# polli-labs/linnaeus

Hardware: AMD Instinct MI355X
Metric: images/sec (train fwd+bwd) mFormerV1_sm 3x224x224 (higher is better)
Workload: dtype bf16; 1 GPU; mFormerV1_sm train step (forward + 4-task CE loss + backward + AdamW (one HIP launch)), bf16 operands / fp32 accumulate+residual, batch 256/GPU, 3x224x224 synthetic, DropPath 0.2, gradient checkpointing off; per_gpu_batch=256, global_batch=256, parallelism=dp1, grad_mode=direct

## Files before the change

include/lnx.h:

```cpp
#ifndef LNX_H
#define LNX_H
#include <stdint.h>

#ifdef __cplusplus
extern "C" {
#endif

#define LNX_F32 0
#define LNX_BF16 1

const char* lnx_last_error(void);
int lnx_version(void);
int lnx_device_cus(void);
int lnx_set_cu_margin(int cus);

typedef struct lnx_rowmap {
    int group, pad, off;
} lnx_rowmap;

enum { LNX_ACT_NONE = 0, LNX_ACT_GELU = 1, LNX_ACT_RELU = 2, LNX_ACT_GELU_BWD = 3, LNX_ACT_RELU_BWD = 4,
       LNX_ACT_GELU_D = 5, LNX_ACT_MUL_AUX = 6 };
enum { LNX_ADDR_PLAIN = 0, LNX_ADDR_PATCH2 = 1 };

typedef struct lnx_gemm_args {
// ... 9 lines not shown
    int a_mode, Hin, Win, Cin;
    int c_mode;
    lnx_rowmap c_map;
    const float* bias;
    void* c2;
    int64_t ldc2;
    int act;
    const void* aux;
    int64_t ldaux;
    const float* gamma;
    const float* rowscale;
    int rows_per_sample;
    const float* res;
    int64_t ldres;
    void* c8;
    int64_t ldc8;
    void* c8_scales;
} lnx_gemm_args;

int lnx_gemm_nt(const lnx_gemm_args* args, void* stream);

#define LNX_GEMM_GROUP_MAX 8
int lnx_gemm_nt_group_ok(const lnx_gemm_args* problems, int n, int accumulate);
int lnx_gemm_nt_group(const lnx_gemm_args* problems, int n, int accumulate, void* stream);

enum { LNX_NT_KERNEL_NONE = 0, LNX_NT_KERNEL_V1 = 1 , LNX_NT_KERNEL_V2 = 2 ,
       LNX_NT_KERNEL_SKINNY = 3 , LNX_NT_KERNEL_V4 = 4 ,
       LNX_NT_KERNEL_FP8 = 6 , LNX_NT_KERNEL_V7 = 7 ,
       LNX_NT_KERNEL_MX8 = 8 , LNX_NT_KERNEL_V9 = 9 ,
       LNX_NT_KERNEL_EXPERIMENT = 15 , LNX_NT_KERNEL_KINDS = 16 };
int lnx_last_nt_kernel(void);
int64_t lnx_nt_kernel_launches(int kind);
int lnx_nt_dispatch(const lnx_gemm_args* args);

int lnx_amax(const void* x, int x_dtype, int64_t ldx, int rows, int cols, float* amax, void* stream);
int lnx_quantize_fp8(const void* x, int x_dtype, int64_t ldx, int rows, int cols, const float* amax, void* y, int64_t ldy, float* scale_out, void* stream);
int lnx_gemm_nt_fp8(const lnx_gemm_args* args, const float* a_scale, const float* w_scale, void* stream);

int lnx_quantize_mxfp8(const void* x, int x_dtype, int64_t ldx, int rows, int cols, void* y, int64_t ldy, void* scales, void* stream);
int lnx_gemm_nt_mxfp8(const lnx_gemm_args* args, const void* a_scales, const void* w_scales, void* stream);

typedef struct lnx_wgrad_args {
    int dtype;
    int M, N, K;
    const void* dY;
    int64_t lddy;
    const void* A;
    int64_t lda;
    int a_mode, Hin, Win, Cin;
    float* dW;
    int64_t lddw;
    int k_perm_c;
    float* db;
    int splits;
    int k_store;
    float* ws;
    int64_t ws_floats;
    int defer;
} lnx_wgrad_args;
#define LNX_TN_WS_FLOATS (256 * (256 * 128 + 256))

int lnx_gemm_tn(const lnx_wgrad_args* args, void* stream);
int lnx_gemm_tn_flush(void* stream);
int lnx_gemm_tn_discard(void);


// ... 52 lines not shown
    void* dx2_8_scales;
    int64_t lddx2_8;
    int defer;
} lnx_ln_bwd_args;
int lnx_layernorm_bwd(const lnx_ln_bwd_args* args, void* stream);
int lnx_layernorm_bwd_flush(void* stream);
int lnx_layernorm_bwd_discard(void);

enum { LNX_LN_COLS_NONE = 0 , LNX_LN_COLS_ATOMICS = 1 ,
       LNX_LN_COLS_WORKSPACE = 2  };
typedef struct lnx_ln_launch {
    int G;
    int V;
    int pair;
    int full;
    int mx;
    int grid;
    int cols;
    int slices;
} lnx_ln_launch;
int lnx_layernorm_fwd_query(const lnx_ln_args* args, lnx_ln_launch* out);
int lnx_layernorm_bwd_query(const lnx_ln_bwd_args* args, lnx_ln_launch* out);

typedef struct lnx_dwconv_args {
    int B, H, W, C;
    const void* x;
    int x_dtype;
    const float* w49;
    const float* bias;
    int flip;
    const float* res;
    void* y;
    int y_dtype;
} lnx_dwconv_args;
int lnx_dwconv7_fwd(const lnx_dwconv_args* args, void* stream);

typedef struct lnx_dwconv_wgrad_args {
    int B, H, W, C;
    const void* x;
    int x_dtype;
    const void* dy;
    int dy_dtype;
    float* dw;
    float* db;
} lnx_dwconv_wgrad_args;
int lnx_dwconv7_wgrad(const lnx_dwconv_wgrad_args* args, void* stream);

enum { LNX_ROPE_COS = 0, LNX_ROPE_ROTATE = 1 };
int lnx_rope_cos_table(const float* freqs , int heads, int H, int W, float* cos_out ,
                       float* dsin_out ,
                       void* stream);
int lnx_rope_cos_table_hd(const float* freqs, int heads, int head_dim, int H, int W, float* cos_out, float* dsin_out, void* stream);
int lnx_rope_cossin_table_hd(const float* freqs, int heads, int head_dim, int H, int W, float* cos_out, float* sin_out, float* dsin_out, void* stream);
#define LNX_ROPE_TABLES_MAX 24
typedef struct {
    const float* freqs;
    float* cos_out;
    float* dsin_out;
    int heads, H, W;
    int head_dim;
    int rope_mode;
    float* sin_out;
} lnx_rope_table;
int lnx_rope_cos_tables(const lnx_rope_table* tables, int n, void* stream);
int64_t lnx_attn_bwd_ws_floats(int B, int N, int heads);
int64_t lnx_attn_bwd_ws_floats_hd(int B, int N, int heads, int head_dim);
// ... 448 lines not shown
    void* ln_out;
    float* mean;
    float* rstd;
} lnx_convmlp_args;
int lnx_convmlp_fwd(const lnx_convmlp_args* args, void* stream);

typedef struct lnx_convmlp_bwd_args {
    int dtype, M, C;
    const float* g;
    const void* ln;
    const void* z;
    const void* w1;
    const float* b1;
    const void* w2t;
    const void* w1t;
    const float* gamma;
    const float* rowscale;
    int rows_per_sample;
    void* act;
    void* dh;
    void* dz;
    void* dln;
    float* dgamma;
    const void* y;
    const float* ln_w;
    const float* mean;
    const float* rstd;
    float* d_ln_w;
    float* d_ln_b;
    float* ws;
    int64_t ws_floats;
    int dz_plain;
    int ln_defer;
} lnx_convmlp_bwd_args;
int lnx_convmlp_bwd(const lnx_convmlp_bwd_args* args, void* stream);
int64_t lnx_convmlp_bwd_ws_floats(int C, int M);


#define LNX_MAX_META 8
#define LNX_MAX_TASKS 16
typedef struct lnx_mformer_cfg {
    int dtype;
    int batch, img_h, img_w, in_chans;
    int dims[4];
    int conv_depths[2];
    int rope_depths[2];
    int rope_heads[2];
    int mlp_hidden[2];
    int n_meta;
    int meta_dims[LNX_MAX_META];
    int only_last_cls;
    int n_tasks;
    int task_classes[LNX_MAX_TASKS];
    int inference;
    int recompute;
    int fp8;
    int rope_mode;
} lnx_mformer_cfg;

typedef struct lnx_plan lnx_plan;
int lnx_plan_create(const lnx_mformer_cfg* cfg, lnx_plan** out);
void lnx_plan_destroy(lnx_plan* p);
int64_t lnx_plan_workspace_bytes(const lnx_plan* p);
int lnx_plan_num_params(const lnx_plan* p);
const char* lnx_plan_param_name(const lnx_plan* p, int i);
int64_t lnx_plan_param_numel(const lnx_plan* p, int i);
// ... 28 lines not shown
```

linnaeus_amd/_lib.py:

```python
from __future__ import annotations

import ctypes as C
import os

_HERE = os.path.dirname(os.path.abspath(__file__))
LIB_PATH = os.environ.get("LNX_LIB_PATH") or os.path.join(_HERE, "liblnx_hip.so")

F32, BF16 = 0, 1
ACT_NONE, ACT_GELU, ACT_RELU, ACT_GELU_BWD, ACT_RELU_BWD, ACT_GELU_D, ACT_MUL_AUX = 0, 1, 2, 3, 4, 5, 6
TN_WS_FLOATS = 256 * (256 * 128 + 256)
ADDR_PLAIN, ADDR_PATCH2 = 0, 1


class LnxError(RuntimeError):
    pass


class RowMap(C.Structure):
    _fields_ = [("group", C.c_int), ("pad", C.c_int), ("off", C.c_int)]


class GemmArgs(C.Structure):
    _fields_ = [
        ("dtype", C.c_int), ("M", C.c_int), ("N", C.c_int), ("K", C.c_int),
# ... 199 lines not shown
            _lib.lnx_resize_coeffs.argtypes = [C.c_int, C.c_int, C.c_int, C.c_void_p, C.c_void_p]
            _lib.lnx_preprocess_scratch_bytes.argtypes = [C.POINTER(PreprocessImage), C.c_int, C.c_int, C.c_int, C.c_int]
            _lib.lnx_preprocess_scratch_bytes.restype = C.c_int64
            _lib.lnx_preprocess.argtypes = [C.POINTER(PreprocessArgs), C.c_void_p]
            _lib.lnx_preprocess.restype = C.c_int
        if hasattr(_lib, "lnx_meta_mask"):
            _lib.lnx_meta_mask.argtypes = [C.POINTER(MetaMaskArgs), C.c_void_p]
            _lib.lnx_meta_mask.restype = C.c_int
        if hasattr(_lib, "lnx_layernorm_fwd_query"):
            _lib.lnx_layernorm_fwd_query.argtypes = [C.POINTER(LnArgs), C.POINTER(LnLaunch)]
            _lib.lnx_layernorm_bwd_query.argtypes = [C.POINTER(LnBwdArgs), C.POINTER(LnLaunch)]
        older = bool(os.environ.get("LNX_LIB_PATH")) and os.environ.get("LNX_LIB_OLDER") == "1"
        for name in EXPORTS:
            if not hasattr(_lib, name) and not older:
                raise LnxError(f"{LIB_PATH} does not export {name}; rebuild it")
    return _lib


def check(rc: int, what: str) -> None:
    if rc != 0:
        raise LnxError(f"{what} failed (rc={rc}): {lib().lnx_last_error().decode()}")


AUG_CLAMP, AUG_POSTERIZE, AUG_SOLARIZE, AUG_SOLARIZE_ADD, AUG_INVERT, AUG_BRIGHTNESS, AUG_CONTRAST = range(7)

NT_KERNEL_NONE, NT_KERNEL_V1, NT_KERNEL_V2, NT_KERNEL_SKINNY, NT_KERNEL_V4, NT_KERNEL_FP8, NT_KERNEL_V7, NT_KERNEL_MX8, NT_KERNEL_V9, NT_KERNEL_EXPERIMENT = 0, 1, 2, 3, 4, 6, 7, 8, 9, 15

ROPE_COS, ROPE_ROTATE = 0, 1

ATTN_KERNEL_NONE, ATTN_KERNEL_RES4, ATTN_KERNEL_RES8, ATTN_KERNEL_TILED4, ATTN_KERNEL_TILED8 = range(5)

EXPORTS = [
    "lnx_last_error", "lnx_version", "lnx_device_cus", "lnx_set_cu_margin",
    "lnx_gemm_nt", "lnx_last_nt_kernel", "lnx_nt_kernel_launches", "lnx_nt_dispatch", "lnx_gemm_tn", "lnx_gemm_tn_flush", "lnx_gemm_tn_discard", "lnx_amax", "lnx_quantize_fp8", "lnx_gemm_nt_fp8", "lnx_quantize_mxfp8", "lnx_gemm_nt_mxfp8", "lnx_dropout_mul", "lnx_dropout_residual", "lnx_plan_dropout_bytes", "lnx_plan_set_dropout", "lnx_plan_attn_dropout_bytes", "lnx_plan_set_attn_dropout",
    "lnx_layernorm_fwd", "lnx_layernorm_bwd", "lnx_layernorm_bwd_flush", "lnx_layernorm_bwd_discard", "lnx_layernorm_fwd_query", "lnx_layernorm_bwd_query",
    "lnx_dwconv7_fwd", "lnx_dwconv7_wgrad",
    "lnx_gemm_nt_group_ok", "lnx_gemm_nt_group", "lnx_rope_cos_table", "lnx_rope_cos_table_hd", "lnx_rope_cossin_table_hd", "lnx_rope_cos_tables", "lnx_attn_bwd_ws_floats", "lnx_attn_bwd_ws_floats_hd", "lnx_attn_fwd", "lnx_attn_bwd", "lnx_attn_bwd_flush", "lnx_attn_bwd_discard", "lnx_attn_dispatch", "lnx_last_attn_kernel", "lnx_last_attn_bwd_launches",
    "lnx_im2col_stem", "lnx_scale_cast", "lnx_layerscale_bwd", "lnx_layerscale_apply_wgrad", "lnx_fill_rows", "lnx_colsum_rows",
    "lnx_agg2_fwd", "lnx_agg2_bwd", "lnx_pack_meta", "lnx_meta_heads_supported", "lnx_meta_heads_fwd", "lnx_meta_heads_bwd", "lnx_meta_heads_bwd_part_floats", "lnx_prep_weights", "lnx_prep_blocks", "lnx_softce", "lnx_softce_multi", "lnx_stem_fwd", "lnx_stem_fwd_ok", "lnx_adamw_blocks", "lnx_grad_sumsq", "lnx_adamw_step", "lnx_ademamix_step", "lnx_muon_layout", "lnx_muon_step", "lnx_muon_launches", "lnx_gradnorm_sumsq", "lnx_gradnorm_update",
    "lnx_metrics_table_sizes", "lnx_metrics_update", "lnx_predict", "lnx_resize_taps", "lnx_resize_coeffs", "lnx_preprocess_scratch_bytes", "lnx_preprocess", "lnx_hier_loss_fwd", "lnx_hier_loss_bwd",
    "lnx_mix_rows", "lnx_mix_meta", "lnx_meta_mask",
    "lnx_aug_pointwise", "lnx_aug_saturation", "lnx_aug_rowstat", "lnx_aug_rescale", "lnx_aug_affine", "lnx_aug_stencil", "lnx_erase_rects", "lnx_u8hwc_to_f32chw",
    "lnx_convmlp_supported", "lnx_convmlp_fwd", "lnx_convmlp_bwd", "lnx_convmlp_bwd_ws_floats",
    "lnx_plan_create", "lnx_plan_destroy", "lnx_plan_workspace_bytes", "lnx_plan_num_params", "lnx_plan_param_name",
    "lnx_plan_param_numel", "lnx_plan_num_drop_calls", "lnx_plan_logits_numel", "lnx_plan_logits_offset", "lnx_plan_logits_ld",
    "lnx_plan_bind", "lnx_plan_forward", "lnx_plan_backward", "lnx_plan_backward_into", "lnx_plan_segment_params", "lnx_plan_profile_begin", "lnx_plan_profile_end", "lnx_plan_profile_begin_spans", "lnx_plan_profile_end_ex", "lnx_plan_set_wgrad_stream", "lnx_plan_set_meta_stream",
]


class MetaHeadArgs(C.Structure):
    _fields_ = [
        ("B", C.c_int), ("C", C.c_int), ("dim", C.c_int), ("off", C.c_int),
        ("meta", C.c_void_p), ("meta_width", C.c_int), ("eps", C.c_float),
        ("w0", C.c_void_p), ("ldw0", C.c_int), ("b0", C.c_void_p), ("ln0_w", C.c_void_p), ("ln0_b", C.c_void_p),
        ("w1", C.c_void_p), ("ldw1", C.c_int), ("b1", C.c_void_p), ("ln1_w", C.c_void_p), ("ln1_b", C.c_void_p),
        ("w2", C.c_void_p), ("ldw2", C.c_int), ("b2", C.c_void_p), ("ln2_w", C.c_void_p), ("ln2_b", C.c_void_p),
        ("t0", C.c_void_p), ("h0", C.c_void_p), ("x", C.c_void_p), ("h1", C.c_void_p), ("n1", C.c_void_p), ("h2", C.c_void_p),
        ("m0", C.c_void_p), ("r0", C.c_void_p), ("m1", C.c_void_p), ("r1", C.c_void_p), ("m2", C.c_void_p), ("r2", C.c_void_p),
        ("tok", C.c_void_p), ("tok_row_stride", C.c_int64), ("tok_row_offset", C.c_int64),
    ]


class MetaHeadBwdArgs(C.Structure):
    _fields_ = [
        ("B", C.c_int), ("C", C.c_int), ("dim", C.c_int),
        ("g", C.c_void_p), ("g_row_stride", C.c_int64), ("g_row_offset", C.c_int64),
        ("w1t", C.c_void_p), ("ldw1t", C.c_int), ("w2t", C.c_void_p), ("ldw2t", C.c_int),
# ... 24 lines not shown
        ("M", C.c_int), ("C", C.c_int),
        ("dy", C.c_void_p), ("dy_dtype", C.c_int), ("lddy", C.c_int64), ("dy_map", RowMap),
        ("x", C.c_void_p), ("x_dtype", C.c_int), ("ldx", C.c_int64), ("x_map", RowMap),
        ("w", C.c_void_p), ("mean", C.c_void_p), ("rstd", C.c_void_p),
        ("gin", C.c_void_p), ("ldgin", C.c_int64),
        ("dx", C.c_void_p), ("dx_dtype", C.c_int), ("lddx", C.c_int64),
        ("dw", C.c_void_p), ("db", C.c_void_p), ("relu_mask", C.c_int),
        ("ws", C.c_void_p), ("ws_floats", C.c_int64),
        ("dx2", C.c_void_p), ("dx2_dtype", C.c_int), ("lddx2", C.c_int64), ("dx2_rowscale", C.c_void_p), ("dx2_rows_per_sample", C.c_int),
        ("dx2_8", C.c_void_p), ("dx2_8_scales", C.c_void_p), ("lddx2_8", C.c_int64),
        ("defer", C.c_int),
    ]


LN_COLS_NONE, LN_COLS_ATOMICS, LN_COLS_WORKSPACE = range(3)


class LnLaunch(C.Structure):
    _fields_ = [("G", C.c_int), ("V", C.c_int), ("pair", C.c_int), ("full", C.c_int), ("mx", C.c_int), ("grid", C.c_int), ("cols", C.c_int), ("slices", C.c_int)]


class RopeTable(C.Structure):
    _fields_ = [
        ("freqs", C.c_void_p), ("cos_out", C.c_void_p), ("dsin_out", C.c_void_p),
        ("heads", C.c_int), ("H", C.c_int), ("W", C.c_int), ("head_dim", C.c_int),
        ("rope_mode", C.c_int), ("sin_out", C.c_void_p),
    ]


class DwconvArgs(C.Structure):
    _fields_ = [
        ("B", C.c_int), ("H", C.c_int), ("W", C.c_int), ("C", C.c_int),
        ("x", C.c_void_p), ("x_dtype", C.c_int), ("w49", C.c_void_p), ("bias", C.c_void_p),
        ("flip", C.c_int), ("res", C.c_void_p), ("y", C.c_void_p), ("y_dtype", C.c_int),
    ]


class DwconvWgradArgs(C.Structure):
    _fields_ = [
        ("B", C.c_int), ("H", C.c_int), ("W", C.c_int), ("C", C.c_int),
        ("x", C.c_void_p), ("x_dtype", C.c_int), ("dy", C.c_void_p), ("dy_dtype", C.c_int),
        ("dw", C.c_void_p), ("db", C.c_void_p),
    ]


class AttnArgs(C.Structure):
    _fields_ = [
        ("dtype", C.c_int), ("B", C.c_int), ("N", C.c_int), ("E", C.c_int), ("heads", C.c_int),
        ("qkv", C.c_void_p), ("cos_tab", C.c_void_p), ("o", C.c_void_p), ("lse", C.c_void_p),
        ("drop_mask", C.c_void_p), ("drop_inv_keep", C.c_float), ("head_dim", C.c_int),
        ("rope_mode", C.c_int), ("sin_tab", C.c_void_p),
    ]


class AttnBwdArgs(C.Structure):
    _fields_ = [
        ("dtype", C.c_int), ("B", C.c_int), ("N", C.c_int), ("E", C.c_int), ("heads", C.c_int),
        ("qkv", C.c_void_p), ("cos_tab", C.c_void_p), ("o", C.c_void_p), ("lse", C.c_void_p),
        ("d_o", C.c_void_p), ("dqkv", C.c_void_p), ("freq_ws", C.c_void_p), ("delta", C.c_void_p),
        ("drop_mask", C.c_void_p), ("drop_inv_keep", C.c_float),
        ("dsin_tab", C.c_void_p), ("dfreqs", C.c_void_p), ("defer_freqs", C.c_int), ("head_dim", C.c_int),
        ("rope_mode", C.c_int), ("sin_tab", C.c_void_p), ("grid_w", C.c_int),
    ]


class PrepDesc(C.Structure):
    _fields_ = [
        ("src", C.c_void_p), ("dst", C.c_void_p), ("dst_t", C.c_void_p),
        ("rows", C.c_int), ("cols", C.c_int), ("ld", C.c_int), ("ld_t", C.c_int),
        ("P", C.c_int), ("mode", C.c_int), ("block_start", C.c_int),
    ]


PREP_CAST, PREP_CONV_PERM, PREP_DW49 = 0, 1, 2


class ConvMlpArgs(C.Structure):
    _fields_ = [
        ("dtype", C.c_int), ("M", C.c_int), ("C", C.c_int),
        ("ln", C.c_void_p), ("w1", C.c_void_p), ("b1", C.c_void_p), ("w2", C.c_void_p), ("b2", C.c_void_p),
        ("gamma", C.c_void_p), ("rowscale", C.c_void_p), ("rows_per_sample", C.c_int),
        ("x", C.c_void_p), ("out", C.c_void_p), ("z", C.c_void_p),
        ("y", C.c_void_p), ("ln_w", C.c_void_p), ("ln_b", C.c_void_p), ("ln_eps", C.c_float), ("ln_out", C.c_void_p),
        ("mean", C.c_void_p), ("rstd", C.c_void_p),
    ]


class ConvMlpBwdArgs(C.Structure):
    _fields_ = [
        ("dtype", C.c_int), ("M", C.c_int), ("C", C.c_int),
        ("g", C.c_void_p), ("ln", C.c_void_p), ("z", C.c_void_p), ("w1", C.c_void_p), ("b1", C.c_void_p),
        ("w2t", C.c_void_p), ("w1t", C.c_void_p), ("gamma", C.c_void_p), ("rowscale", C.c_void_p), ("rows_per_sample", C.c_int),
        ("act", C.c_void_p), ("dh", C.c_void_p), ("dz", C.c_void_p), ("dln", C.c_void_p), ("dgamma", C.c_void_p),
        ("y", C.c_void_p), ("ln_w", C.c_void_p), ("mean", C.c_void_p), ("rstd", C.c_void_p), ("d_ln_w", C.c_void_p), ("d_ln_b", C.c_void_p),
        ("ws", C.c_void_p), ("ws_floats", C.c_int64),
        ("dz_plain", C.c_int), ("ln_defer", C.c_int),
    ]


class StemArgs(C.Structure):
    _fields_ = [("x", C.c_void_p), ("w", C.c_void_p), ("bias", C.c_void_p), ("ln_w", C.c_void_p), ("ln_b", C.c_void_p), ("patches", C.c_void_p),
                ("pre", C.c_void_p), ("y", C.c_void_p), ("mean", C.c_void_p), ("rstd", C.c_void_p), ("B", C.c_int), ("Cin", C.c_int), ("H", C.c_int),
                ("W", C.c_int), ("Cout", C.c_int), ("eps", C.c_float)]


class MixArgs(C.Structure):
    _fields_ = [
        ("x", C.c_void_p), ("perm", C.c_void_p), ("valid", C.c_void_p), ("out", C.c_void_p),
        ("B", C.c_int), ("row", C.c_int64), ("H", C.c_int), ("W", C.c_int), ("lam", C.c_float),
        ("h0", C.c_int), ("h1", C.c_int), ("w0", C.c_int), ("w1", C.c_int), ("mode", C.c_int),
    ]


META_MASK_MAX_COMPONENTS = 32


class MetaMaskArgs(C.Structure):
    _fields_ = [
        ("aux", C.c_void_p), ("mask", C.c_void_p), ("out_aux", C.c_void_p), ("out_mask", C.c_void_p),
        ("B", C.c_int), ("D", C.c_int), ("bounds", C.c_void_p), ("ncomp", C.c_int), ("ncombo", C.c_int),
        ("combo_bits", C.c_void_p), ("combo_thr", C.c_void_p), ("draws", C.c_void_p), ("combo_idx", C.c_void_p),
        ("p_full", C.c_float), ("p_partial", C.c_float), ("partial_on", C.c_int), ("row_bits", C.c_uint), ("row_full", C.c_int),
        ("counts", C.c_void_p), ("row_combo", C.c_void_p),
    ]
```

linnaeus_amd/csrc/api.cpp:

```cpp
#include <hip/hip_runtime.h>
#include <stdarg.h>
#include <stdio.h>
#include <stdlib.h>
#include <string.h>

#include <atomic>
#include <mutex>

#include "../../include/lnx.h"

static thread_local char g_err[1024] = "";

void lnx_set_error(const char* fmt, ...) {
    va_list ap;
    va_start(ap, fmt);
    vsnprintf(g_err, sizeof(g_err), fmt, ap);
    va_end(ap);
}

extern "C" const char* lnx_last_error(void) { return g_err; }
extern "C" int lnx_version(void) { return 109; }
extern "C" int lnx_device_cus(void) {
    int dev = 0;
    if (hipGetDevice(&dev) != hipSuccess) return -1;
    hipDeviceProp_t prop;
    if (hipGetDeviceProperties(&prop, dev) != hipSuccess) return -1;
    return prop.multiProcessorCount;
}

static std::atomic<int> g_cu_margin{-1};
int persistent_cus(int cus) {
    int m = g_cu_margin.load(std::memory_order_relaxed);
    if (m < 0) {
        const char* e = getenv("LNX_CU_MARGIN");
        m = e ? atoi(e) : 0;
        if (m < 0) m = 0;
        g_cu_margin.store(m, std::memory_order_relaxed);
    }
    const int room = cus - m;
    return room < 8 ? 8 : room;
}
void set_cu_margin(int m) { g_cu_margin.store(m < 0 ? 0 : m, std::memory_order_relaxed); }
bool tile_sched_static() {
    const char* e = getenv("LNX_TILE_SCHED");
    return e && strcmp(e, "static") == 0;
}
int tile_slot_of(hipStream_t st) {
    static std::mutex mu;
    static hipStream_t known[64];
    static int n = 0;
    std::lock_guard<std::mutex> lock(mu);
    for (int i = 0; i < n; ++i)
        if (known[i] == st) return i;
    if (n < 64) {
// ... 23 lines not shown
```

linnaeus_amd/csrc/convmlp.hip:

```cpp
#include <stdlib.h>

#include "common.hpp"
#include "../../include/lnx.h"

namespace {

struct CmP {
    const unsigned char* ln;
    const unsigned char* w1;
    const unsigned char* w2;
    const unsigned char* w2t;
    const unsigned char* w1t;
    const unsigned char* zin;
    const float* b1;
    const float* b2;
    const float* gamma;
    const float* rowscale;
    const float* x;
    const float* g;
    float* out;
    unsigned char* z;
    unsigned char* act;
    unsigned char* dh;
    unsigned char* dz;
// ... 207 lines not shown
#pragma unroll
        for (int b = 0; b < GB; ++b)
#pragma unroll
            for (int mt = 0; mt < MT; ++mt) mfma16(o[c0 + b][mt], wf[bt & 1][b], pf[mt][ks2]);
    }
}

__device__ __forceinline__ uint4 pack8(const f32x4_t& lo, const f32x4_t& hi) {
    Vec16<bf16_t> v;
#pragma unroll
    for (int j = 0; j < 4; ++j) {
        v.set(j, lo[j]);
        v.set(4 + j, hi[j]);
    }
    return v.raw;
}

__device__ __forceinline__ float g_sum(float v) {
    v += __shfl_xor(v, 16, 64);
    v += __shfl_xor(v, 32, 64);
    return v;
}
template <int CTRL> __device__ __forceinline__ float dpp_get(float v) {
    return __builtin_bit_cast(float, __builtin_amdgcn_update_dpp(0, __builtin_bit_cast(int, v), CTRL, 0xf, 0xf, false));
}
__device__ __forceinline__ float row16_sum(float v) {
    v += dpp_get<0xB1>(v);
    v += dpp_get<0x4E>(v);
    v += dpp_get<0x141>(v);
    v += dpp_get<0x140>(v);
    return v;
}
template <int NK>
__device__ __forceinline__ void ln_row_frags(uint4 (&xf)[NK], const float* w, const float* b, int g, float eps, float& mu, float& rs) {
    constexpr float invC = 1.0f / (float)Geo<NK>::C;
    float v[NK][8];
    float sum = 0.f;
#pragma unroll
    for (int ks = 0; ks < NK; ++ks) {
        Vec16<bf16_t> t;
        t.raw = xf[ks];
#pragma unroll
        for (int j = 0; j < 8; ++j) v[ks][j] = t.get(j);
        sum += ((v[ks][0] + v[ks][1]) + (v[ks][2] + v[ks][3])) + ((v[ks][4] + v[ks][5]) + (v[ks][6] + v[ks][7]));
    }
    mu = g_sum(sum) * invC;
    float sq = 0.f;
#pragma unroll
    for (int ks = 0; ks < NK; ++ks)
#pragma unroll
        for (int j = 0; j < 8; ++j) {
            v[ks][j] -= mu;
            sq = fmaf(v[ks][j], v[ks][j], sq);
        }
    rs = 1.0f / sqrtf(fmaf(g_sum(sq), invC, eps));
#pragma unroll
    for (int ks = 0; ks < NK; ++ks) {
        const int c = ks * 32 + 8 * g;
        const float4 w0 = *reinterpret_cast<const float4*>(w + c), w1 = *reinterpret_cast<const float4*>(w + c + 4);
        const float4 b0 = *reinterpret_cast<const float4*>(b + c), b1 = *reinterpret_cast<const float4*>(b + c + 4);
        const float wv[8] = {w0.x, w0.y, w0.z, w0.w, w1.x, w1.y, w1.z, w1.w};
        const float bv[8] = {b0.x, b0.y, b0.z, b0.w, b1.x, b1.y, b1.z, b1.w};
        Vec16<bf16_t> o;
#pragma unroll
        for (int j = 0; j < 8; ++j) o.set(j, fmaf(v[ks][j] * rs, wv[j], bv[j]));
        xf[ks] = o.raw;
    }
}
template <int NK>
struct LnRow {
    uint2 yr[Geo<NK>::CT];
    float mu, rs;
};
template <int NK>
__device__ __forceinline__ void ln_bwd_fetch(LnRow<NK>& r, const CmP& p, int m, int g) {
    constexpr int C = Geo<NK>::C;
    const int mc = m < p.M ? m : p.M - 1;
#pragma unroll
    for (int ct = 0; ct < Geo<NK>::CT; ++ct) r.yr[ct] = *reinterpret_cast<const uint2*>(p.y + ((int64_t)mc * C + ct * 16 + 4 * g) * 2);
    r.mu = p.mean[mc];
    r.rs = p.rstd[mc];
}
template <int NK, int MT, int MTI>
__device__ __forceinline__ void ln_bwd_rows(const CmP& p, const f32x4_t (&dl)[Geo<NK>::CT][MT], const LnRow<NK>& row, int m, int s, int g, const float* lnws,
                                            float* dls) {
    constexpr int C = Geo<NK>::C;
    constexpr int CT = Geo<NK>::CT;
    constexpr float invC = 1.0f / (float)C;
    const bool mv = m < p.M;
    const int mc = mv ? m : p.M - 1;
    const uint2 (&yr)[CT] = row.yr;
    const float mu = row.mu, rs = row.rs;
    float xh[CT][4], gv[CT][4];
    float s1 = 0.f, s2 = 0.f;
#pragma unroll
    for (int ct = 0; ct < CT; ++ct) {
        const int c = ct * 16 + 4 * g;
        const float4 w4 = *reinterpret_cast<const float4*>(lnws + c);
        const float wv[4] = {w4.x, w4.y, w4.z, w4.w};
        const bf16_t* yh = reinterpret_cast<const bf16_t*>(&yr[ct]);
// ... 160 lines not shown
            if (p.z) {
                uint2 zz;
                bf16_t* zh = reinterpret_cast<bf16_t*>(&zz);
                zh[0] = (bf16_t)z0; zh[1] = (bf16_t)z1; zh[2] = (bf16_t)z2; zh[3] = (bf16_t)z3;
                *reinterpret_cast<uint2*>(p.z + ((int64_t)m * C + c) * 2) = zz;
            }
            *reinterpret_cast<float4*>(p.out + (int64_t)m * C + c) =
                make_float4(xr.x + rs * gm.x * z0, xr.y + rs * gm.y * z1, xr.z + rs * gm.z * z2, xr.w + rs * gm.w * z3);
        }
    }
    CM_T(7);
#ifdef CM_STAMP
    if (blockIdx.x == gridDim.x / 2 && threadIdx.x == 0)
        for (int i = 0; i < 8; ++i) g_cm_stamp[i] = tsum[i];
#endif
}
#ifdef CM_STAMP
extern "C" int lnx_dbg_convmlp_stamps(unsigned long long* out8) { return (int)hipMemcpyFromSymbol(out8, HIP_SYMBOL(g_cm_stamp), 64); }
#endif

template <int NK, int MT, int NW, bool ST, bool LNB, bool DG>
__global__ __launch_bounds__(64 * NW) void convmlp_bwd_kernel(const CmP p) {
    constexpr int C = Geo<NK>::C;
    constexpr int CT = Geo<NK>::CT;
    constexpr int PART = Geo<NK>::PART;
    constexpr int STAGE = 3 * PART;
    constexpr int NCH = 4 * C / 64;
    constexpr int NLD = 12 * NK / NW;
    extern __shared__ __attribute__((aligned(16))) unsigned char smem[];
    float* b1s = reinterpret_cast<float*>(smem + 2 * STAGE);
    float* dgs = b1s + 4 * C;
    float* lws = dgs + C;
    float* dls = lws + C;

    const int lane = threadIdx.x & 63;
    const int wave = __builtin_amdgcn_readfirstlane(threadIdx.x >> 6);
    const int s = lane & 15, g = lane >> 4;
    const int m_base = blockIdx.x * (16 * NW * MT) + wave * (16 * MT);
    const uint32_t lds0 = (uint32_t)(uintptr_t)(__attribute__((address_space(3))) unsigned char*)smem;

    for (int i = threadIdx.x; i < 4 * C; i += 64 * NW) b1s[i] = p.b1[i];
    for (int i = threadIdx.x; i < C; i += 64 * NW) {
        dgs[i] = 0.f;
        if constexpr (LNB) {
            lws[i] = p.lnw[i];
            dls[i] = dls[C + i] = 0.f;
        }
    }
    __syncthreads();

    uint4 xf[MT][NK], zf[MT][NK];
    bool mvalid[MT];
#pragma unroll
    for (int mt = 0; mt < MT; ++mt) {
        int m = m_base + mt * 16 + s;
        mvalid[mt] = m < p.M;
        if (!mvalid[mt]) m = p.M - 1;
        const float rs = p.rowscale ? p.rowscale[m / p.rps] : 1.0f;
        float4 g0v[NK], g1v[NK], a0v[NK], a1v[NK];
        uint4 zraw[NK];
#pragma unroll
        for (int ks = 0; ks < NK; ++ks) {
            const int c = ks * 32 + 8 * g;
            xf[mt][ks] = ld16(p.ln + ((int64_t)m * C + c) * 2);
            g0v[ks] = *reinterpret_cast<const float4*>(p.g + (int64_t)m * C + c);
            g1v[ks] = *reinterpret_cast<const float4*>(p.g + (int64_t)m * C + c + 4);
            a0v[ks] = *reinterpret_cast<const float4*>(p.gamma + c);
            a1v[ks] = *reinterpret_cast<const float4*>(p.gamma + c + 4);
            if constexpr (DG) zraw[ks] = ld16(p.zin + ((int64_t)m * C + c) * 2);
        }
#pragma unroll
        for (int ks = 0; ks < NK; ++ks) {
            const int c = ks * 32 + 8 * g;
            const float4 g0 = g0v[ks], g1 = g1v[ks], a0 = a0v[ks], a1 = a1v[ks];
            Vec16<bf16_t> zin, dzv, dzs;
            if constexpr (DG) zin.raw = zraw[ks];
            const float gv[8] = {g0.x, g0.y, g0.z, g0.w, g1.x, g1.y, g1.z, g1.w};
            const float av[8] = {a0.x, a0.y, a0.z, a0.w, a1.x, a1.y, a1.z, a1.w};
#pragma unroll
            for (int j = 0; j < 8; ++j) {
                const float sg = rs * gv[j];
                dzv.set(j, sg * av[j]);
                dzs.set(j, p.dz_plain ? sg : sg * av[j]);
                if constexpr (DG) {
                    const float dgp = mvalid[mt] ? sg * zin.get(j) : 0.f;
                    float t = dgp;
                    t += __shfl_xor(t, 1, 64);
                    t += __shfl_xor(t, 2, 64);
                    t += __shfl_xor(t, 4, 64);
                    t += __shfl_xor(t, 8, 64);
                    if (s == 0) atomicAdd(&dgs[c + j], t);
                }
            }
            zf[mt][ks] = dzv.raw;
            st16(p.dz + ((int64_t)m * C + c) * 2, dzs.raw);
        }
    }
    f32x4_t dl[CT][MT];
#pragma unroll
    for (int ct = 0; ct < CT; ++ct)
#pragma unroll
        for (int mt = 0; mt < MT; ++mt) dl[ct][mt] = f32x4_t{0.f, 0.f, 0.f, 0.f};
    LnRow<NK> lrow;
    if constexpr (LNB) ln_bwd_fetch<NK>(lrow, p, m_base + s, g);

    __syncthreads();
    dma_nmajor<NK, NW>(smem, p.w1, 0, wave, lane);
    dma_nmajor<NK, NW>(smem + PART, p.w2t, 0, wave, lane);
    dma_cmajor<NK, NW>(smem + 2 * PART, p.w1t, 0, wave, lane);
    for (int j = 0; j < NCH; ++j) {
        const int stg = j & 1;
        __builtin_amdgcn_s_barrier();
        if (j + 1 < NCH) {
            unsigned char* nx = smem + (stg ^ 1) * STAGE;
            dma_nmajor<NK, NW>(nx, p.w1, 64 * (j + 1), wave, lane);
            dma_nmajor<NK, NW>(nx + PART, p.w2t, 64 * (j + 1), wave, lane);
            dma_cmajor<NK, NW>(nx + 2 * PART, p.w1t, 64 * (j + 1), wave, lane);
            asm volatile("s_waitcnt vmcnt(%0)" ::"n"(NLD) : "memory");
        } else {
            asm volatile("s_waitcnt vmcnt(0)" ::: "memory");
        }
        __builtin_amdgcn_s_barrier();
        const uint32_t st = lds0 + stg * STAGE;
        f32x4_t h[4][MT], da[4][MT];
        prod_nmajor_pipe<NK, MT>(h, st, s, g, xf);
        prod_nmajor_pipe<NK, MT>(da, st + PART, s, g, zf);
        f32x4_t bv[4];
        const uint32_t ba = lds0 + 2 * STAGE + (uint32_t)((64 * j + 8 * g) * 4);
        CM_DS_READ128(bv[0], ba, 0);
        CM_DS_READ128(bv[1], ba, 16);
        CM_DS_READ128(bv[2], ba, 128);
        CM_DS_READ128(bv[3], ba, 144);
        asm volatile("s_waitcnt lgkmcnt(0)" ::: "memory");
        __builtin_amdgcn_sched_barrier(0);
#pragma unroll
        for (int mt = 0; mt < MT; ++mt)
#pragma unroll
// ... 553 lines not shown
    CmP q = p;
    q.tile_slot = tile_sched_static() ? -1 : tile_slot_of(st);
    hipLaunchKernelGGL((convmlp_bwd_res_kernel<NK, MT, ST, LNB, DG>), dim3(grid), dim3(512), lds, st, q);
    return LNB ? reduce_ln_partials(p, grid, st) : 0;
}
template <int NK, int MT>
int launch_bwd_res(const CmP& p, hipStream_t st) {
    if (p.zin == nullptr) {
        if (p.y) return p.act ? launch_bwd_res_t<NK, MT, true, true, false>(p, st) : launch_bwd_res_t<NK, MT, false, true, false>(p, st);
        return p.act ? launch_bwd_res_t<NK, MT, true, false, false>(p, st) : launch_bwd_res_t<NK, MT, false, false, false>(p, st);
    }
    if (p.y) return p.act ? launch_bwd_res_t<NK, MT, true, true, true>(p, st) : launch_bwd_res_t<NK, MT, false, true, true>(p, st);
    return p.act ? launch_bwd_res_t<NK, MT, true, false, true>(p, st) : launch_bwd_res_t<NK, MT, false, false, true>(p, st);
}

template <int NK, int MT, int NW, bool LNF>
int launch_fwd_t(const CmP& p, hipStream_t st) {
    const size_t lds = 3 * 2 * Geo<NK>::PART + 4 * Geo<NK>::C * sizeof(float);
    static bool attr = false;
    if (!attr) {
        (void)hipFuncSetAttribute(reinterpret_cast<const void*>(&convmlp_fwd_kernel<NK, MT, NW, LNF>), hipFuncAttributeMaxDynamicSharedMemorySize, (int)lds);
        attr = true;
    }
    hipLaunchKernelGGL((convmlp_fwd_kernel<NK, MT, NW, LNF>), dim3(cdiv(p.M, 16 * NW * MT)), dim3(64 * NW), lds, st, p);
    return 0;
}
template <int NK, int MT, int NW>
int launch_fwd(const CmP& p, hipStream_t st) {
    return p.y ? launch_fwd_t<NK, MT, NW, true>(p, st) : launch_fwd_t<NK, MT, NW, false>(p, st);
}

template <int NK, int MT, int NW, bool ST, bool LNB, bool DG>
int launch_bwd_t(const CmP& p, hipStream_t st) {
    const size_t lds = 2 * 3 * Geo<NK>::PART + 8 * Geo<NK>::C * sizeof(float);
    static bool attr = false;
    if (!attr) {
        (void)hipFuncSetAttribute(reinterpret_cast<const void*>(&convmlp_bwd_kernel<NK, MT, NW, ST, LNB, DG>), hipFuncAttributeMaxDynamicSharedMemorySize, (int)lds);
        attr = true;
    }
    static_assert(MT == 1, "bwd_grid() assumes 16-row wave tiles in the streamed-weight backward");
    const int grid = bwd_grid(p.C, p.M);
    if (LNB && (int64_t)grid * 2 * p.C > p.part_floats) return -1;
    hipLaunchKernelGGL((convmlp_bwd_kernel<NK, MT, NW, ST, LNB, DG>), dim3(grid), dim3(64 * NW), lds, st, p);
    return LNB ? reduce_ln_partials(p, grid, st) : 0;
}
template <int NK, int MT, int NW>
int launch_bwd(const CmP& p, hipStream_t st) {
    if (p.zin == nullptr) {
        if (p.y) return p.act ? launch_bwd_t<NK, MT, NW, true, true, false>(p, st) : launch_bwd_t<NK, MT, NW, false, true, false>(p, st);
        return p.act ? launch_bwd_t<NK, MT, NW, true, false, false>(p, st) : launch_bwd_t<NK, MT, NW, false, false, false>(p, st);
    }
    if (p.y) return p.act ? launch_bwd_t<NK, MT, NW, true, true, true>(p, st) : launch_bwd_t<NK, MT, NW, false, true, true>(p, st);
    return p.act ? launch_bwd_t<NK, MT, NW, true, false, true>(p, st) : launch_bwd_t<NK, MT, NW, false, false, true>(p, st);
}

}

extern "C" int64_t lnx_convmlp_bwd_ws_floats(int C, int M) {
    if (!lnx_convmlp_supported(LNX_BF16, C) || M <= 0) return 0;
    return (int64_t)bwd_grid(C, M) * 2 * C;
}

extern "C" int lnx_convmlp_supported(int dtype, int C) { return dtype == LNX_BF16 && (C == 32 || C == 64 || C == 96 || C == 128 || C == 192); }

extern "C" int lnx_convmlp_fwd(const lnx_convmlp_args* a, void* stream) {
    LNX_CHECK(a && (a->ln || a->y) && a->w1 && a->w2 && a->b1 && a->b2 && a->gamma && a->x && a->out, "lnx_convmlp_fwd: null operand");
    if (a->y) {
        LNX_CHECK(a->ln_w && a->ln_b && a->ln == nullptr, "lnx_convmlp_fwd: the fused LayerNorm form takes y, ln_w, ln_b and no ln");
        LNX_CHECK((a->mean == nullptr) == (a->ln_out == nullptr) && (a->rstd == nullptr) == (a->ln_out == nullptr) && (a->z == nullptr || a->ln_out != nullptr),
                  "lnx_convmlp_fwd: with y, the outputs ln_out, mean and rstd are written together (what a backward needs) or not at all; z only with them");
    }
    LNX_CHECK(lnx_convmlp_supported(a->dtype, a->C), "lnx_convmlp_fwd: unsupported dtype %d / C %d (bf16, C in {32,64,96,128,192})", a->dtype, a->C);
    LNX_CHECK(a->M > 0, "lnx_convmlp_fwd: empty");
    if (a->rowscale) LNX_CHECK(a->rows_per_sample > 0, "lnx_convmlp_fwd: rowscale needs rows_per_sample");
    CmP p{};
    p.ln = (const unsigned char*)a->ln; p.w1 = (const unsigned char*)a->w1; p.w2 = (const unsigned char*)a->w2;
    p.b1 = a->b1; p.b2 = a->b2; p.gamma = a->gamma; p.rowscale = a->rowscale; p.x = a->x; p.out = a->out; p.z = (unsigned char*)a->z;
    p.M = a->M; p.C = a->C; p.rps = a->rows_per_sample > 0 ? a->rows_per_sample : 1;
    p.y = (const unsigned char*)a->y; p.lnw = a->ln_w; p.lnb = a->ln_b; p.eps = a->ln_eps; p.ln_out = (unsigned char*)a->ln_out; p.mean = a->mean; p.rstd = a->rstd;
    hipStream_t st = (hipStream_t)stream;
    switch (a->C) {
        case 32: launch_fwd_res<1>(p, st); break;
        case 64: launch_fwd_res<2>(p, st); break;
        case 96: launch_fwd_res<3>(p, st); break;
        case 128: if (nw8) launch_fwd<4, 1, 8>(p, st); else launch_fwd<4, 1, 4>(p, st); break;
        case 192: if (nw8) launch_fwd<6, 1, 8>(p, st); else launch_fwd<6, 1, 4>(p, st); break;
    }
    LNX_LAUNCH_CHECK();
    return 0;
}

extern "C" int lnx_convmlp_bwd(const lnx_convmlp_bwd_args* a, void* stream) {
    LNX_CHECK(a && a->g && a->ln && a->w1 && a->w2t && a->w1t && a->b1 && a->gamma && a->dz && a->dln && (a->dgamma || !a->z),
              "lnx_convmlp_bwd: null operand (z may be NULL: dgamma is then not produced here; with z, dgamma is required)");
    LNX_CHECK((a->act == nullptr) == (a->dh == nullptr), "lnx_convmlp_bwd: act and dh must both be given or both be NULL");
    LNX_CHECK(lnx_convmlp_supported(a->dtype, a->C), "lnx_convmlp_bwd: unsupported dtype %d / C %d", a->dtype, a->C);
    LNX_CHECK(a->M > 0, "lnx_convmlp_bwd: empty");
    if (a->rowscale) LNX_CHECK(a->rows_per_sample > 0, "lnx_convmlp_bwd: rowscale needs rows_per_sample");
    if (a->y) LNX_CHECK(a->ln_w && a->mean && a->rstd && a->d_ln_w && a->d_ln_b && a->ws, "lnx_convmlp_bwd: the fused LayerNorm form needs ln_w, mean, rstd, d_ln_w, d_ln_b and ws");
    CmP p{};
    p.y = (const unsigned char*)a->y; p.lnw = a->ln_w; p.mean = const_cast<float*>(a->mean); p.rstd = const_cast<float*>(a->rstd);
    p.part = a->ws; p.part_floats = a->ws_floats; p.dlnw = a->d_ln_w; p.dlnb = a->d_ln_b; p.ln_defer = a->ln_defer;
    p.g = a->g; p.ln = (const unsigned char*)a->ln; p.zin = (const unsigned char*)a->z; p.w1 = (const unsigned char*)a->w1;
    p.w2t = (const unsigned char*)a->w2t; p.w1t = (const unsigned char*)a->w1t; p.b1 = a->b1; p.gamma = a->gamma; p.rowscale = a->rowscale;
    p.act = (unsigned char*)a->act; p.dh = (unsigned char*)a->dh; p.dz = (unsigned char*)a->dz; p.dln = (unsigned char*)a->dln; p.dgamma = a->dgamma;
    p.M = a->M; p.C = a->C; p.rps = a->rows_per_sample > 0 ? a->rows_per_sample : 1;
    p.dz_plain = a->dz_plain != 0;
    hipStream_t st = (hipStream_t)stream;
    int rc = 0;
    switch (a->C) {
        case 32: rc = launch_bwd_res<1, 2>(p, st); break;
        case 64: rc = launch_bwd_res<2, 1>(p, st); break;
        case 96: rc = launch_bwd_res<3, 1>(p, st); break;
        case 128: rc = nw8 ? launch_bwd<4, 1, 8>(p, st) : launch_bwd<4, 1, 4>(p, st); break;
        case 192: rc = nw8 ? launch_bwd<6, 1, 8>(p, st) : launch_bwd<6, 1, 4>(p, st); break;
    }
    LNX_CHECK(rc == 0, "lnx_convmlp_bwd: ws too small for the LayerNorm partial sums (M=%d C=%d ws_floats=%lld)", a->M, a->C, (long long)a->ws_floats);
    LNX_LAUNCH_CHECK();
    return 0;
}
```

linnaeus_amd/csrc/dwconv.hip:

```cpp
#include "common.hpp"
#include "../../include/lnx.h"
#include "dwconv_mfma.hpp"

namespace {

constexpr int TH = 8, TW = 16, CB = 32;
constexpr int IH = TH + 6, IW = TW + 6;
constexpr int NV = IH * IW * (CB / 4);
constexpr int NPRE = (NV + 255) / 256;
constexpr int NDY = TH * TW * (CB / 4) / 256;

struct DwP {
    const void* x;
    const float* w49;
    const float* bias;
    const float* res;
    void* y;
    int B, H, W, C;
    int flip;
    int tiles_h, tiles_w, cblocks;
    int tiles_per_wg;
};

template <typename TX> struct Raw4;
// ... 225 lines not shown
#pragma unroll
            for (int k = 0; k < NDY; ++k) *reinterpret_cast<float4*>(dyt + 4 * (threadIdx.x + 256 * k)) = widen(pdy[k]);
            __syncthreads();
        }
    }
    float* red = tile;
#pragma unroll
    for (int pass = 0; pass < 2; ++pass) {
        const int tbeg = pass * 25;
        const int tcnt = pass == 0 ? 25 : 24;
#pragma unroll
        for (int t = 0; t < 25; ++t) {
            if (t < tcnt) red[(r * 25 + t) * CB + cl] = acc[tbeg + t];
            else if (pass == 1) red[(r * 25 + t) * CB + cl] = accb;
        }
        __syncthreads();
        for (int i = threadIdx.x; i < 25 * CB; i += 256) {
            const int t = i / CB, c = i % CB;
            float s = 0.f;
#pragma unroll
            for (int rr = 0; rr < 8; ++rr) s += red[(rr * 25 + t) * CB + c];
            if (t < tcnt) atomicAdd(p.dw + (int64_t)(c0 + c) * 49 + tbeg + t, s);
            else if (pass == 1 && p.db) atomicAdd(p.db + c0 + c, s);
        }
        __syncthreads();
    }
}

}

extern "C" int lnx_dwconv7_fwd(const lnx_dwconv_args* a, void* stream) {
    LNX_CHECK(a && a->x && a->w49 && a->y, "lnx_dwconv7_fwd: null operand");
    LNX_CHECK(a->B > 0 && a->H > 0 && a->W > 0 && a->C > 0 && a->C % CB == 0, "lnx_dwconv7_fwd: bad shape B=%d H=%d W=%d C=%d (C %% 32)", a->B, a->H, a->W, a->C);
    if (lnx_dwconv_mfma_enabled() && (a->x_dtype == LNX_BF16 || a->y_dtype == LNX_BF16) && !(a->res && a->y_dtype != LNX_F32))
        return lnx_dwconv7_mfma_fwd(a, (hipStream_t)stream);
    DwP p;
    p.x = a->x; p.w49 = a->w49; p.bias = a->bias; p.res = a->res; p.y = a->y;
    p.B = a->B; p.H = a->H; p.W = a->W; p.C = a->C; p.flip = a->flip;
    p.tiles_h = cdiv(a->H, TH); p.tiles_w = cdiv(a->W, TW); p.cblocks = a->C / CB;
    const int64_t ntile = (int64_t)a->B * p.tiles_h * p.tiles_w;
    int per = p.tiles_h * p.tiles_w;
    while (per > 1 && (int64_t)cdiv(ntile, per) * p.cblocks < 3 * 256) per = (per + 1) / 2;
    p.tiles_per_wg = per;
    const int64_t grid = (int64_t)cdiv(ntile, per) * p.cblocks;
    LNX_CHECK(grid < (1ll << 31), "lnx_dwconv7_fwd: grid too large");
    hipStream_t st = (hipStream_t)stream;
    const int code = a->x_dtype * 2 + a->y_dtype + (a->flip ? 4 : 0);
#define DWL(TX, TY, F) hipLaunchKernelGGL((dwconv7_kernel<TX, TY, F>), dim3((int)grid), dim3(256), 0, st, p)
    switch (code) {
        case 0: DWL(float, float, false); break;
        case 1: DWL(float, bf16_t, false); break;
        case 2: DWL(bf16_t, float, false); break;
        case 3: DWL(bf16_t, bf16_t, false); break;
        case 4: DWL(float, float, true); break;
        case 5: DWL(float, bf16_t, true); break;
        case 6: DWL(bf16_t, float, true); break;
        case 7: DWL(bf16_t, bf16_t, true); break;
        default: LNX_CHECK(false, "lnx_dwconv7_fwd: bad dtypes");
    }
#undef DWL
    LNX_LAUNCH_CHECK();
    return 0;
}

extern "C" int lnx_dwconv7_wgrad(const lnx_dwconv_wgrad_args* a, void* stream) {
    LNX_CHECK(a && a->x && a->dy && a->dw, "lnx_dwconv7_wgrad: null operand");
    LNX_CHECK(a->B > 0 && a->H > 0 && a->W > 0 && a->C > 0 && a->C % CB == 0, "lnx_dwconv7_wgrad: bad shape");
    if (lnx_dwconv_mfma_enabled() && (a->x_dtype == LNX_BF16 || a->dy_dtype == LNX_BF16)) return lnx_dwconv7_mfma_wgrad(a, (hipStream_t)stream);
    DwWgP p;
    p.x = a->x; p.dy = a->dy; p.dw = a->dw; p.db = a->db;
    p.B = a->B; p.H = a->H; p.W = a->W; p.C = a->C;
    p.tiles_h = cdiv(a->H, TH); p.tiles_w = cdiv(a->W, TW); p.cblocks = a->C / CB;
    p.ntile = a->B * p.tiles_h * p.tiles_w;
    int walkers = 768 / p.cblocks;
    if (walkers < 1) walkers = 1;
    if (walkers > p.ntile) walkers = p.ntile;
    const int grid = walkers * p.cblocks;
    hipStream_t st = (hipStream_t)stream;
    const int code = a->x_dtype * 2 + a->dy_dtype;
    switch (code) {
        case 0: hipLaunchKernelGGL((dwconv7_wgrad_kernel<float, float>), dim3(grid), dim3(256), 0, st, p); break;
        case 1: hipLaunchKernelGGL((dwconv7_wgrad_kernel<float, bf16_t>), dim3(grid), dim3(256), 0, st, p); break;
        case 2: hipLaunchKernelGGL((dwconv7_wgrad_kernel<bf16_t, float>), dim3(grid), dim3(256), 0, st, p); break;
        case 3: hipLaunchKernelGGL((dwconv7_wgrad_kernel<bf16_t, bf16_t>), dim3(grid), dim3(256), 0, st, p); break;
        default: LNX_CHECK(false, "lnx_dwconv7_wgrad: bad dtypes");
    }
    LNX_LAUNCH_CHECK();
    return 0;
}
```

linnaeus_amd/csrc/dwconv_mfma.hip:

```cpp
#include "common.hpp"
#include "dwconv_mfma.hpp"
#include <stdlib.h>

namespace {

typedef uint32_t u32;
typedef __attribute__((ext_vector_type(4))) u32 u32x4;

__device__ __forceinline__ __amdgpu_buffer_rsrc_t tile_rsrc(const void* base) {
    const uint64_t a = reinterpret_cast<uint64_t>(base);
    const u32 hi = (u32)__builtin_amdgcn_readfirstlane((int)(a >> 32)), lo = (u32)__builtin_amdgcn_readfirstlane((int)(u32)a);
    const uint64_t u = (uint64_t)hi << 32 | lo;
    return __builtin_amdgcn_make_buffer_rsrc(reinterpret_cast<void*>(u), 0, 0x7fffffff, 0x00020000);
}
constexpr u32 OOB = 0x80000000u;
__device__ __forceinline__ uint4 buf_ld16(__amdgpu_buffer_rsrc_t r, u32 voff, u32 soff) {
    const u32x4 v = __builtin_amdgcn_raw_buffer_load_b128(r, voff, (u32)__builtin_amdgcn_readfirstlane((int)soff), 0);
    return make_uint4(v[0], v[1], v[2], v[3]);
}
__device__ __forceinline__ void buf_st16(__amdgpu_buffer_rsrc_t r, u32 voff, uint4 v) {
    __builtin_amdgcn_raw_buffer_store_b128(u32x4{v.x, v.y, v.z, v.w}, r, voff, 0, 0);
}
constexpr int CPW = 2;

__device__ __forceinline__ u32 pack2(float a, float b) {
    typedef __attribute__((ext_vector_type(2))) __bf16 bf16x2_t;
    bf16x2_t v = {(bf16_t)a, (bf16_t)b};
    return __builtin_bit_cast(u32, v);
}

template <typename T, int NTHR, int CBM, int ROWS, int CPAIRS, int PITCH, int PLANE>
struct Stage {
    static constexpr int CH = 16 / sizeof(T);
    static constexpr int NCG = CBM / CH;
    static constexpr int NU = ROWS * CPAIRS * NCG;
    static constexpr int NPU = (NU + NTHR - 1) / NTHR;
    uint4 p0[NPU], p1[NPU];
    u32 goff[NPU];
    int rc[NPU];
    int cgoff;
    static_assert(NTHR % NCG == 0, "one channel group per thread");

    __device__ __forceinline__ void init(int W, int C) {
#pragma unroll
        for (int k = 0; k < NPU; ++k) {
            const int u = threadIdx.x + NTHR * k;
            const int cg = u % NCG, cp = (u / NCG) % CPAIRS, row = u / (NCG * CPAIRS);
            const bool on = u < NU;
            goff[k] = on ? (u32)((row * W + 2 * cp) * C + cg * CH) * (u32)sizeof(T) : 0u;
            cgoff = cg * CH * PLANE;
            rc[k] = on ? (row | (2 * cp) << 8) : -1;
        }
    }

// ... 75 lines not shown
    pair = (blockIdx.x >> 4) * 8 + (within & 7);
    half = within >> 3;
}

template <int NTHR> __device__ __forceinline__ void zero_lds(char* base, int bytes) {
    for (int i = threadIdx.x * 16; i < bytes; i += NTHR * 16) *reinterpret_cast<uint4*>(base + i) = make_uint4(0u, 0u, 0u, 0u);
}

__device__ __forceinline__ f32x4_t mfma32(const uint4& a, const uint4& b, f32x4_t acc) {
    return __builtin_amdgcn_mfma_f32_16x16x32_bf16(__builtin_bit_cast(bf16x8_t, a), __builtin_bit_cast(bf16x8_t, b), acc, 0, 0, 0);
}

constexpr int FT = 1024, FCB = 32;
constexpr int MT = 14;
constexpr int MI = MT + 6;
constexpr int XROWS = MI + 2;
constexpr int XPITCH = 48;
constexpr int XPLANE = XROWS * XPITCH + 16;
constexpr int X_BYTES = FCB * XPLANE;
template <typename TY> struct OutT {
    static constexpr int PITCH = FCB * sizeof(TY) + (sizeof(TY) == 2 ? 8 : 16);
    static constexpr int PARTS = FCB * sizeof(TY) / 16;
    static constexpr int NOU = MT * MT * PARTS;
    static constexpr int NPO = (NOU + FT - 1) / FT;
    static constexpr int BYTES = MT * MT * PITCH;
};

struct MfP {
    const void* x;
    const float* w49;
    const float* bias;
    const float* res;
    void* y;
    int B, H, W, C;
    int tiles_h, tiles_w, tiles_per_wg, ntile, chunks;
};

struct TileAt {
    int b, h0, w0;
};
struct TileCursor {
    int b, h0, w0;
    __device__ __forceinline__ void step(int H, int W, int th, int tw) {
        w0 += tw;
        if (w0 >= W) {
            w0 = 0;
            h0 += th;
            if (h0 >= H) {
                h0 = 0;
                ++b;
            }
        }
    }
};
__device__ __forceinline__ TileAt tile_at(int t, int tiles_h, int tiles_w, int th, int tw) {
    TileAt q;
    const int t2 = t / tiles_w;
    q.w0 = (t % tiles_w) * tw;
    q.h0 = (t2 % tiles_h) * th;
    q.b = t2 / tiles_h;
    return q;
}

#ifdef DW_STAMP
__device__ unsigned long long g_dwm_stamp[8];
#define DWM_T(i) do { __builtin_amdgcn_sched_barrier(0); unsigned long long t_; asm volatile("s_memtime %0\n\ts_waitcnt lgkmcnt(0)" : "=s"(t_) :: "memory"); \
                      __builtin_amdgcn_sched_barrier(0); tsum[i] += t_ - tlast; tlast = t_; } while (0)
#else
#define DWM_T(i) do { } while (0)
#endif

template <typename TX, typename TY, bool FLIP>
__global__ __launch_bounds__(FT) void dwconv7_mfma_kernel(const MfP p) {
    extern __shared__ __attribute__((aligned(16))) char smem[];
    typedef Stage<TX, FT, FCB, MI, MI / 2, XPITCH, XPLANE> St;
    typedef OutT<TY> Ot;
    char* xt = smem;
    char* ot = smem + X_BYTES;
    const int cb = blockIdx.x / p.chunks;
    const int t_begin = (blockIdx.x % p.chunks) * p.tiles_per_wg;
    const int t_end = min(p.ntile, t_begin + p.tiles_per_wg);
    const int c0 = cb * FCB;
    const int wave = threadIdx.x >> 6, lane = threadIdx.x & 63;
    const int n = lane & 15, g = lane >> 4;
    const TX* xg = reinterpret_cast<const TX*>(p.x) + c0;

    St sa;
    sa.init(p.W, p.C);
    TileCursor cq, cq2;
    {
        const TileAt q = tile_at(t_begin, p.tiles_h, p.tiles_w, MT, MT);
        cq.b = q.b; cq.h0 = q.h0; cq.w0 = q.w0;
        cq2 = cq;
        sa.issue(xg, cq2.b, cq2.h0 - 3, cq2.w0 - 3, p.H, p.W, p.C, true);
        cq2.step(p.H, p.W, MT, MT);
    }
    zero_lds<FT>(xt, X_BYTES);
    float* wl = reinterpret_cast<float*>(ot);
    for (int i = threadIdx.x; i < 49 * FCB; i += FT) wl[i] = p.w49[(int64_t)(i / FCB) * p.C + c0 + (i % FCB)];
    __syncthreads();
    uint4 tz[CPW][7];
#pragma unroll
    for (int c = 0; c < CPW; ++c)
#pragma unroll
        for (int ky = 0; ky < 7; ++ky) {
            u32 wd[4];
// ... 67 lines not shown
            for (int c = 0; c < CPW; ++c) bf[ky][c] = *reinterpret_cast<const uint4*>(xb + c * XPLANE + ky * XPITCH);
#pragma unroll
        for (int ky = 0; ky < 7; ++ky) {
            if (ky + AHEAD < 7) {
#pragma unroll
                for (int c = 0; c < CPW; ++c) bf[(ky + AHEAD) % (AHEAD + 1)][c] = *reinterpret_cast<const uint4*>(xb + c * XPLANE + (ky + AHEAD) * XPITCH);
            }
            if (ky < St::NLOAD) sa.issue_one(ft, ky, p.H, p.W, p.C);
            __builtin_amdgcn_sched_barrier(0);
#pragma unroll
            for (int c = 0; c < CPW; ++c) acc[c] = mfma32(tz[c][ky], bf[ky % (AHEAD + 1)][c], acc[c]);
            __builtin_amdgcn_sched_barrier(0);
        }
        static_assert(St::NLOAD <= 7, "one load per kernel row");
        DWM_T(1);
        if (n < MT) {
#pragma unroll
            for (int i = 0; i < 4; ++i) {
                const int m = 4 * g + i;
                if (m < MT) {
                    char* o = ow + (n * MT + m) * Ot::PITCH;
                    if constexpr (sizeof(TY) == 2)
                        *reinterpret_cast<u32*>(o) = pack2(acc[0][i] + bv[0], acc[1][i] + bv[1]);
                    else
                        *reinterpret_cast<float2*>(o) = make_float2(acc[0][i] + bv[0], acc[1][i] + bv[1]);
                }
            }
        }
        DWM_T(2);
        __syncthreads();
        DWM_T(3);
        {
            const __amdgpu_buffer_rsrc_t yr = tile_rsrc(reinterpret_cast<const TY*>(p.y) + tile0);
#pragma unroll
            for (int k = 0; k < Ot::NPO; ++k) {
                const char* o = ot + ol[k];
                if constexpr (sizeof(TY) == 2) {
                    const uint2 lo = *reinterpret_cast<const uint2*>(o), hi = *reinterpret_cast<const uint2*>(o + 8);
#ifndef DW_NOSTORE
                    buf_st16(yr, go[k], make_uint4(lo.x, lo.y, hi.x, hi.y));
#else
                    if (lo.x == 0x12345678u) buf_st16(yr, go[k], make_uint4(lo.x, lo.y, hi.x, hi.y));
#endif
                } else {
                    float4 v = *reinterpret_cast<const float4*>(o);
                    if (p.res) {
                        v.x += __builtin_bit_cast(float, rv[k].x); v.y += __builtin_bit_cast(float, rv[k].y);
                        v.z += __builtin_bit_cast(float, rv[k].z); v.w += __builtin_bit_cast(float, rv[k].w);
                    }
                    buf_st16(yr, go[k], make_uint4(__builtin_bit_cast(u32, v.x), __builtin_bit_cast(u32, v.y), __builtin_bit_cast(u32, v.z), __builtin_bit_cast(u32, v.w)));
                }
            }
        }
        DWM_T(4);
        if (t + 1 < t_end) sa.commit(xt);
        DWM_T(5);
        __syncthreads();
        DWM_T(6);
    }
#ifdef DW_STAMP
    if (blockIdx.x == gridDim.x / 2 && threadIdx.x == 0)
        for (int i = 0; i < 8; ++i) g_dwm_stamp[i] = tsum[i];
#endif
}
#ifdef DW_STAMP
extern "C" int lnx_dbg_dwconv_mfma_stamps(unsigned long long* out8) { return (int)hipMemcpyFromSymbol(out8, HIP_SYMBOL(g_dwm_stamp), 64); }
#endif

constexpr int WT = 512, WCB = 16;
constexpr int WH = 14, WW = 28;
constexpr int WXR = WH + 6, WXC = WW + 6;
constexpr int WX_PITCH = 80;
constexpr int WX_PLANE = WXR * WX_PITCH + 16;
constexpr int WX_BYTES = WCB * WX_PLANE;
constexpr int WD_ROWS = WXR + 7;
constexpr int WD_PITCH = 64;
constexpr int WD_PLANE = WD_ROWS * WD_PITCH + 16;
constexpr int WD_BYTES = WCB * WD_PLANE;

struct MwP {
    const void* x;
    const void* dy;
    float* dw;
// ... 82 lines not shown
            const uint4 a = make_uint4(__builtin_amdgcn_alignbit(d[1], d[0], shift), __builtin_amdgcn_alignbit(d[2], d[1], shift),
                                       __builtin_amdgcn_alignbit(d[3], d[2], shift), __builtin_amdgcn_alignbit(d[4], d[3], shift));
            acc = mfma32(a, bq[r & 1], acc);
            __builtin_amdgcn_sched_barrier(0);
        }
        __syncthreads();
        if (more) {
            sx.commit(xt);
            sd.commit(dt + 7 * WD_PITCH);
            sd.add_channel_sums(dbs);
            __syncthreads();
        }
    }
#pragma unroll
    for (int i = 0; i < 4; ++i) {
        const int m = 4 * g + i;
        const int kx = m & 7;
        if ((m >> 3) == ch && kx < 7 && kk < 7) atomicAdd(p.dw + (int64_t)(c0 + CPW * wave + ch) * 49 + kk * 7 + kx, acc[i]);
    }
    if (p.db) {
        const int cg = threadIdx.x % Sd::NCG;
#pragma unroll
        for (int j = 0; j < Sd::CH; ++j) atomicAdd(&dbl[cg * Sd::CH + j], dbs[j]);
        __syncthreads();
        if (threadIdx.x < WCB) atomicAdd(p.db + c0 + threadIdx.x, dbl[threadIdx.x]);
    }
}

template <typename K> int set_lds(K kernel, int bytes) {
    LNX_HIP(hipFuncSetAttribute(reinterpret_cast<const void*>(kernel), hipFuncAttributeMaxDynamicSharedMemorySize, bytes));
    return 0;
}

template <typename TX, typename TY, bool FLIP> int launch_fwd(const MfP& p, int grid, hipStream_t st) {
    const int lds = X_BYTES + OutT<TY>::BYTES;
    static bool ready = false;
    if (!ready) {
        if (int rc = set_lds(dwconv7_mfma_kernel<TX, TY, FLIP>, lds)) return rc;
        ready = true;
    }
    hipLaunchKernelGGL((dwconv7_mfma_kernel<TX, TY, FLIP>), dim3(grid), dim3(FT), lds, st, p);
    return 0;
}

template <typename TX, typename TDY> int launch_wgrad(const MwP& p, int grid, hipStream_t st) {
    const int lds = WX_BYTES + WD_BYTES + WCB * (int)sizeof(float);
    static bool ready = false;
    if (!ready) {
        if (int rc = set_lds(dwconv7_mfma_wgrad_kernel<TX, TDY>, lds)) return rc;
        ready = true;
    }
    hipLaunchKernelGGL((dwconv7_mfma_wgrad_kernel<TX, TDY>), dim3(grid), dim3(WT), lds, st, p);
    return 0;
}

int cus() {
    const int n = device_cus();
    return persistent_cus(n > 0 ? n : 256);
}

}

bool lnx_dwconv_mfma_enabled() {
    static const bool on = getenv("LNX_DWCONV_VALU") == nullptr;
    return on;
}

int lnx_dwconv7_mfma_fwd(const lnx_dwconv_args* a, hipStream_t st) {
    MfP p;
    p.x = a->x; p.w49 = a->w49; p.bias = a->bias; p.res = a->res; p.y = a->y;
    p.B = a->B; p.H = a->H; p.W = a->W; p.C = a->C;
    const int code = a->x_dtype * 2 + a->y_dtype + (a->flip ? 4 : 0);
    p.tiles_h = cdiv(a->H, MT); p.tiles_w = cdiv(a->W, MT);
    const int64_t ntile = (int64_t)a->B * p.tiles_h * p.tiles_w;
    LNX_CHECK(ntile < (1ll << 31), "lnx_dwconv7_fwd: too many tiles");
    p.ntile = (int)ntile;
    const int cblocks = a->C / FCB;
    int chunks = cus() / cblocks;
    if (chunks < 1) chunks = 1;
    if (chunks > p.ntile) chunks = p.ntile;
    p.tiles_per_wg = cdiv(p.ntile, chunks);
    p.chunks = cdiv(p.ntile, p.tiles_per_wg);
    const int grid = p.chunks * cblocks;
    LNX_CHECK(!(a->res && a->y_dtype != LNX_F32), "lnx_dwconv7_fwd: a residual needs an fp32 output");
    int rc = 0;
    switch (code) {
        case 1: rc = launch_fwd<float, bf16_t, false>(p, grid, st); break;
        case 2: rc = launch_fwd<bf16_t, float, false>(p, grid, st); break;
        case 3: rc = launch_fwd<bf16_t, bf16_t, false>(p, grid, st); break;
        case 5: rc = launch_fwd<float, bf16_t, true>(p, grid, st); break;
        case 6: rc = launch_fwd<bf16_t, float, true>(p, grid, st); break;
        case 7: rc = launch_fwd<bf16_t, bf16_t, true>(p, grid, st); break;
        default: LNX_CHECK(false, "lnx_dwconv7_fwd: the MFMA path needs a bf16 operand");
    }
    if (rc) return rc;
    LNX_LAUNCH_CHECK();
    return 0;
}

int lnx_dwconv7_mfma_wgrad(const lnx_dwconv_wgrad_args* a, hipStream_t st) {
    MwP p;
    p.x = a->x; p.dy = a->dy; p.dw = a->dw; p.db = a->db;
    p.B = a->B; p.H = a->H; p.W = a->W; p.C = a->C;
    p.tiles_h = cdiv(a->H, WH); p.tiles_w = cdiv(a->W, WW);
    const int64_t ntile = (int64_t)a->B * p.tiles_h * p.tiles_w;
    LNX_CHECK(ntile < (1ll << 31), "lnx_dwconv7_wgrad: too many tiles");
    p.ntile = (int)ntile;
    const int groups = a->C / (2 * WCB);
    int walkers = cus() / groups;
    if (walkers < 1) walkers = 1;
    if (walkers > p.ntile) walkers = p.ntile;
    p.per = cdiv(p.ntile, walkers);
    walkers = cdiv(p.ntile, p.per);
    p.nwalk = walkers;
    const int grid = 16 * cdiv(walkers * groups, 8);
    const int code = a->x_dtype * 2 + a->dy_dtype;
    int rc = 0;
    switch (code) {
        case 1: rc = launch_wgrad<float, bf16_t>(p, grid, st); break;
        case 2: rc = launch_wgrad<bf16_t, float>(p, grid, st); break;
        case 3: rc = launch_wgrad<bf16_t, bf16_t>(p, grid, st); break;
        default: LNX_CHECK(false, "lnx_dwconv7_wgrad: the MFMA path needs a bf16 operand");
    }
    if (rc) return rc;
// ... 4 lines not shown
```

linnaeus_amd/csrc/gemm2.hip:

```cpp
#include "gemm_common.hpp"

namespace lnxg {

#define DS_READ4(dst, addr)                                                                              \
    do {                                                                                                 \
        const uint32_t a_ = (addr);                                                                      \
        asm volatile("ds_read_b128 %0, %1" : "=v"(dst[0]) : "v"(a_) : "memory");                         \
        asm volatile("ds_read_b128 %0, %1 offset:512" : "=v"(dst[1]) : "v"(a_) : "memory");              \
        asm volatile("ds_read_b128 %0, %1 offset:1024" : "=v"(dst[2]) : "v"(a_) : "memory");             \
        asm volatile("ds_read_b128 %0, %1 offset:1536" : "=v"(dst[3]) : "v"(a_) : "memory");             \
    } while (0)

constexpr int BM2 = 256, BN2 = 128;
constexpr int STAGE_BYTES = (BM2 + BN2) * ROWB;
constexpr int NSTAGE = 3;
constexpr int LD_PER_WAVE = (BM2 + BN2) / 8 / 8;

template <bool OUT_F32, bool PATCH, int F>
__global__ __launch_bounds__(512) void gemm_nt_v2_kernel(const GemmP p) {
    typedef bf16_t T;
    constexpr int BK = 64;
    extern __shared__ __attribute__((aligned(16))) unsigned char smem[];

    const int tid = threadIdx.x;
// ... 198 lines not shown
            asm volatile("s_waitcnt vmcnt(4)" ::: "memory");
        } else {
            asm volatile("s_waitcnt vmcnt(0)" ::: "memory");
        }
        asm volatile("s_waitcnt lgkmcnt(0)" ::: "memory");
        __builtin_amdgcn_s_barrier();
        __builtin_amdgcn_sched_barrier(0);
        __builtin_amdgcn_s_setprio(1);
#pragma unroll
        for (int ni = 0; ni < 4; ++ni)
#pragma unroll
            for (int mi = 0; mi < 4; ++mi) Mfma<T>::run(acc0[ni][mi], wf[ni], af0[mi]);
#pragma unroll
        for (int ni = 0; ni < 4; ++ni)
#pragma unroll
            for (int mi = 0; mi < 4; ++mi) Mfma<T>::run(acc1[ni][mi], wf[ni], af1[mi]);
        __builtin_amdgcn_s_setprio(0);
        __builtin_amdgcn_sched_barrier(0);
        if (!(grp && kt + 1 == nk)) __builtin_amdgcn_s_barrier();
    }
    if (F == F_GENERIC) {
        gemm_epilogue<T, OUT_F32>(p, acc0, m0 + wm * 128, n0 + wn * 64, lane);
        gemm_epilogue<T, OUT_F32>(p, acc1, m0 + wm * 128 + 64, n0 + wn * 64, lane);
    } else {
        gemm_epilogue_fast<T, OUT_F32, F>(p, acc0, m0 + wm * 128, n0 + wn * 64, lane);
        gemm_epilogue_fast<T, OUT_F32, F>(p, acc1, m0 + wm * 128 + 64, n0 + wn * 64, lane);
    }
}

constexpr bool nt_v4_carries(bool out_f32, int f) {
    if (out_f32) return f == (F_BIAS | F_RES);
    return f == 0 || f == F_BIAS || f == (F_BIAS | F_C2 | F_GELU) || f == (F_BIAS | F_GELU) || f == F_GELU_BWD;
}
constexpr bool nt_v2_carries(bool out_f32, int f) { return f == F_GENERIC || nt_v4_carries(out_f32, f); }

int launch_nt_v4(const GemmP& p0, int f, bool out_f32, hipStream_t st) {
    GemmP p = p0;
    p.tiles_m = cdiv(p.M, BM4);
    p.tiles_n = p.N / BN4;
    const int grid = p.tiles_m * p.tiles_n;
    return with_nt_form<nt_v4_carries>("gemm_nt_v4", out_f32, f, [&](auto form) {
        using Form = decltype(form);
        return launch_with_lds<gemm_nt_v4_kernel<Form::out_f32, Form::f>>(grid, 512, NST4 * STAGE4, st, p);
    });
}

int launch_nt_v2(const GemmP& p0, int f, bool out_f32, hipStream_t st) {
    GemmP p = p0;
    p.tiles_m = cdiv(p.M, BM2);
    p.tiles_n = cdiv(p.N, BN2);
    const int grid = p.tiles_m * p.tiles_n;
    const size_t lds = NSTAGE * STAGE_BYTES;
    const bool patch = p.a_mode == LNX_ADDR_PATCH2;
    LNX_CHECK(!patch || f == F_GENERIC, "gemm_nt_v2: the 2x2 patch gather is compiled with the generic epilogue only (f = %d)", f);
    return with_nt_form<nt_v2_carries>("gemm_nt_v2", out_f32, f, [&](auto form) {
        using Form = decltype(form);
        if constexpr (Form::f == F_GENERIC) {
            if (patch) return launch_with_lds<gemm_nt_v2_kernel<Form::out_f32, true, Form::f>>(grid, 512, lds, st, p);
        }
        return launch_with_lds<gemm_nt_v2_kernel<Form::out_f32, false, Form::f>>(grid, 512, lds, st, p);
    });
}

constexpr int TBM = 64;

#define DS_READ_TR2(lo, hi, addr, off2)                                                                                  \
    do {                                                                                                                 \
        const uint32_t a_ = (addr);                                                                                      \
        asm volatile("ds_read_b64_tr_b16 %0, %1" : "=v"(lo) : "v"(a_) : "memory");                                       \
        asm volatile("ds_read_b64_tr_b16 %0, %1 offset:%2" : "=v"(hi) : "v"(a_), "i"(off2) : "memory");                 \
    } while (0)

template <int RW, int CW, bool PATCH>
__global__ __launch_bounds__(512) void gemm_tn_v2_kernel(const WgradP p) {
    typedef bf16_t T;
    constexpr int RROW = RW * 2, CROW = CW * 2;
    constexpr int RBYTES = TBM * RROW, CBYTES = TBM * CROW;
    constexpr int STG = RBYTES + CBYTES;
    constexpr int RINS = RBYTES / 1024, CINS = CBYTES / 1024;
    constexpr int NINS = (RINS + CINS) / 8;
    constexpr int WC = CW / 64;
    extern __shared__ __attribute__((aligned(16))) unsigned char smem[];

    const int tid = threadIdx.x;
    const int lane = tid & 63;
    const int wave = __builtin_amdgcn_readfirstlane(tid >> 6);
    const int wr = wave / WC, wc = wave % WC;
    const int s = lane & 15, g = lane >> 4;

    int bid = xcd_remap(blockIdx.x, p.tiles_n * p.tiles_k * p.splits);
// ... 344 lines not shown
```

linnaeus_amd/csrc/gemm3.hip:

```cpp
#include "gemm_common.hpp"

namespace lnxg {

#define V7_READ4(dst, addr)                                                                              \
    do {                                                                                                 \
        const uint32_t a_ = (addr);                                                                      \
        asm volatile("ds_read_b128 %0, %1" : "=v"(dst[0]) : "v"(a_) : "memory");                         \
        asm volatile("ds_read_b128 %0, %1 offset:512" : "=v"(dst[1]) : "v"(a_) : "memory");              \
        asm volatile("ds_read_b128 %0, %1 offset:1024" : "=v"(dst[2]) : "v"(a_) : "memory");             \
        asm volatile("ds_read_b128 %0, %1 offset:1536" : "=v"(dst[3]) : "v"(a_) : "memory");             \
    } while (0)

template <int N> struct IC { static constexpr int value = N; };

constexpr int BM7 = 256, BN7 = 128, BK7 = 64;
constexpr int STAGE7 = (BM7 + BN7) * ROWB;
constexpr int NST7 = 3;
constexpr int PIECES7 = (BM7 + BN7) / 8 / 8;

__device__ __forceinline__ void asm_load16(uint4& d, const void* ptr) {
    asm volatile("global_load_dwordx4 %0, %1, off" : "=v"(d) : "v"(ptr) : "memory");
}
__device__ __forceinline__ void asm_load4(float& d, const void* ptr) {
    asm volatile("global_load_dword %0, %1, off" : "=v"(d) : "v"(ptr) : "memory");
// ... 306 lines not shown
            } else {
                Vec16<T> o;
#pragma unroll
                for (int h = 0; h < 2; ++h) {
#pragma unroll
                    for (int j = 0; j < 8; ++j) o.set(j, v[h * 8 + j]);
                    hc[mi][h] = o.raw;
                }
            }
        }
        pend_row = live ? mbase : -1;
        pend_col = nb;
        if (pend_row >= 0 && (!full || !has_next)) {
#pragma unroll
            for (int sl = 0; sl < NSTORE; ++sl) store_slot(sl, true);
            pend_row = -1;
        }
        if (!has_next) break;
        __builtin_amdgcn_s_barrier();
        pos = next;
        m0 = nm0;
        n0 = nn0;
        src = srcn;
    }
    if (reset_ctr && tid == 0) sched_reset(ctr);
}

constexpr bool nt_v7_carries(bool out_f32, int f) {
    if (out_f32) return f == (F_BIAS | F_RES);
    return f == 0 || f == F_BIAS || f == (F_BIAS | F_C2 | F_GELU) || f == F_GELU_BWD;
}

bool nt_v7_ok(const GemmP& p, int f, bool out_f32) {
    if (p.a_mode == LNX_ADDR_PATCH2) return false;
    if (p.act == LNX_ACT_GELU_D) return false;
    if (p.K % BK7 != 0 || p.K / BK7 < 6) return false;
    if (p.N % 64 != 0) return false;
    const int64_t lim = (int64_t)1 << 31;
    if ((int64_t)p.M * p.lda * 2 >= lim || (int64_t)p.N * p.ldw * 2 >= lim) return false;
    return nt_v7_carries(out_f32, f);
}

int launch_nt_v7(const GemmP& p0, int f, bool out_f32, hipStream_t st) {
    GemmP p = p0;
    p.tiles_m = cdiv(p.M, BM7);
    p.tiles_n = cdiv(p.N, BN7);
    const int ntiles = p.tiles_m * p.tiles_n;
    const int cus = device_cus();
    LNX_CHECK(cus > 0, "gemm_nt_v7: no device");
    const int room = persistent_cus(cus);
    const int grid = ntiles < room ? ntiles : room;
    const size_t lds = NST7 * STAGE7 + 16;
    p.tile_slot = tile_sched_static() ? -1 : tile_slot_of(st);
    const bool deep = p.K / BK7 >= 17;
    return with_nt_form<nt_v7_carries>("gemm_nt_v7", out_f32, f, [&](auto form) {
        using Form = decltype(form);
        if (deep) return launch_with_lds<gemm_nt_v7_kernel<Form::out_f32, Form::f, 8, 8>>(grid, 512, lds, st, p);
        return launch_with_lds<gemm_nt_v7_kernel<Form::out_f32, Form::f, 3, 2>>(grid, 512, lds, st, p);
    });
}

}
```

linnaeus_amd/csrc/gemm5.hip:

```cpp
#include "gemm_common.hpp"

namespace lnxg {

#define V9_READ4(dst, addr)                                                                             \
    do {                                                                                                \
        const uint32_t a_ = (addr);                                                                     \
        asm volatile("ds_read_b128 %0, %1" : "=v"(dst[0]) : "v"(a_) : "memory");                        \
        asm volatile("ds_read_b128 %0, %1 offset:256" : "=v"(dst[1]) : "v"(a_) : "memory");             \
        asm volatile("ds_read_b128 %0, %1 offset:512" : "=v"(dst[2]) : "v"(a_) : "memory");             \
        asm volatile("ds_read_b128 %0, %1 offset:768" : "=v"(dst[3]) : "v"(a_) : "memory");             \
    } while (0)

template <int N> struct IC9 { static constexpr int value = N; };

constexpr int BM9 = 256, BN9 = 256, BK9 = 32, ROWB9 = 64;
constexpr int STAGE9 = (BM9 + BN9) * ROWB9;
constexpr int NST9 = 4;
constexpr int PIECES9 = STAGE9 / 1024 / 8;

__device__ __forceinline__ int key9(int row) { return (row & 16) ? 3 : 0; }

template <bool OUT_F32, int F> struct EpiStores {
    static constexpr int value = 2 * (OUT_F32 ? 16 : 8) + ((F & F_C2) ? 16 : 0);
};
// ... 164 lines not shown
            has_next = next < xcnt;
            reset_ctr = reset_ctr || next == xcnt + xgrid - 1;
        }
        if (has_next) {
            pos_origin(next, nm0, nn0);
#pragma unroll
            for (int j = 0; j < PIECES9; ++j) srcn[j] = piece_offset(j, nm0, nn0);
        }
        for (int kt = 4; kt < nk; ++kt) {
            kstep(kt, IC9<0>(), IC9<0>());
            if (!(grp && kt + 1 == nk && !has_next)) __builtin_amdgcn_s_barrier();
        }
        gemm_epilogue_fast<T, OUT_F32, F>(p, acc0, m0 + wm * 128, n0 + wn * 64, lane);
        gemm_epilogue_fast<T, OUT_F32, F>(p, acc1, m0 + wm * 128 + 64, n0 + wn * 64, lane);
        if (!has_next) break;
        const bool full = m0 + BM9 <= p.M;
        if (!full) asm volatile("s_waitcnt vmcnt(0)" ::: "memory");
        stores_behind = full;
        asm volatile("" ::: "memory");
        pos = next;
        m0 = nm0;
        n0 = nn0;
        src = srcn;
    }
    if (reset_ctr && tid == 0) sched_reset(ctr);
}

constexpr bool nt_v9_carries(bool out_f32, int f) {
    if (out_f32) return f == (F_BIAS | F_RES);
    return f == 0 || f == F_BIAS || f == (F_BIAS | F_C2 | F_GELU) || f == (F_BIAS | F_GELU) || f == F_GELU_BWD;
}

bool nt_v9_ok(const GemmP& p, int f, bool out_f32) {
    if (p.a_mode == LNX_ADDR_PATCH2) return false;
    if (p.N % BN9 != 0 || p.K % BK9 != 0 || p.K / BK9 < 8) return false;
    const int64_t lim = (int64_t)1 << 31;
    if ((int64_t)p.M * p.lda * 2 >= lim || (int64_t)p.N * p.ldw * 2 >= lim) return false;
    return nt_v9_carries(out_f32, f);
}

int launch_nt_v9(const GemmP& p0, int f, bool out_f32, hipStream_t st) {
    GemmP p = p0;
    p.tiles_m = cdiv(p.M, BM9);
    p.tiles_n = p.N / BN9;
    const int ntiles = p.tiles_m * p.tiles_n;
    const int cus = device_cus();
    LNX_CHECK(cus > 0, "gemm_nt_v9: no device");
    const int room = persistent_cus(cus);
    const int grid = ntiles < room ? ntiles : room;
    const size_t lds = NST9 * STAGE9 + 16;
    p.tile_slot = tile_sched_static() ? -1 : tile_slot_of(st);
    return with_nt_form<nt_v9_carries>("gemm_nt_v9", out_f32, f, [&](auto form) {
        using Form = decltype(form);
        return launch_with_lds<gemm_nt_v9_kernel<Form::out_f32, Form::f>>(grid, 512, lds, st, p);
    });
}

}
```

linnaeus_amd/csrc/gemm_common.hpp:

```cpp
#pragma once
#include "common.hpp"
#include "../../include/lnx.h"

namespace lnxg {

constexpr int TILE = 128;
constexpr int ROWB = 128;
constexpr int TILE_BYTES = TILE * ROWB;

struct PatchGeom {
    int Hin, Win, Cin;
};

struct GemmP {
    const unsigned char* A;
    const unsigned char* W;
    unsigned char* C;
    unsigned char* C2;
    const unsigned char* aux;
    const float* bias;
    const float* gamma;
    const float* rowscale;
    const float* res;
    int64_t lda, ldw, ldc, ldc2, ldaux, ldres;
// ... 272 lines not shown
        const bool deriv = (F & F_GELU) && (F & F_C2) && p.act == LNX_ACT_GELU_D;
        if (F & F_C2) {
            float d2[16];
            if (deriv) {
                Gelu<T>::fwd_grad16(v, d2);
            } else {
#pragma unroll
                for (int j = 0; j < 16; ++j) d2[j] = v[j];
            }
            T* c2 = reinterpret_cast<T*>(p.C2) + (m * (int)p.ldc2 + nb);
            Vec16<T> o;
#pragma unroll
            for (int h = 0; h < 16 / EPV; ++h) {
#pragma unroll
                for (int j = 0; j < EPV; ++j) o.set(j, d2[h * EPV + j]);
                st16(c2 + h * EPV, o.raw);
            }
        }
        if ((F & F_GELU) && !deriv) {
            Gelu<T>::fwd16(v);
        }
        if (F & F_GELU_BWD) {
            if (p.act == LNX_ACT_MUL_AUX) {
#pragma unroll
                for (int j = 0; j < 16; ++j) v[j] *= ld[mi][j];
            } else {
                Gelu<T>::mulgrad16(v, ld[mi]);
            }
        }
        if (F & F_RES) {
#pragma unroll
            for (int j = 0; j < 16; ++j) v[j] = fmaf(v[j], rs[mi], ld[mi][j]);
        }
        const int coff = m * (int)p.ldc + nb;
        if (OUT_F32) {
            float* cp = reinterpret_cast<float*>(p.C) + coff;
#pragma unroll
            for (int h = 0; h < 4; ++h) *reinterpret_cast<float4*>(cp + 4 * h) = make_float4(v[4 * h], v[4 * h + 1], v[4 * h + 2], v[4 * h + 3]);
        } else {
            T* cp = reinterpret_cast<T*>(p.C) + coff;
            Vec16<T> o;
#pragma unroll
            for (int h = 0; h < 16 / EPV; ++h) {
#pragma unroll
                for (int j = 0; j < EPV; ++j) o.set(j, v[h * EPV + j]);
                st16(cp + h * EPV, o.raw);
                if (F & F_MXOUT) {
#pragma unroll
                    for (int j = 0; j < EPV; ++j) v[h * EPV + j] = o.get(j);
                }
            }
            if (F & F_MXOUT) {
                float am = 0.f;
#pragma unroll
                for (int j = 0; j < 16; ++j) am = fmaxf(am, fabsf(v[j]));
                am = fmaxf(am, __shfl_xor(am, 16, 64));
                const uint32_t bits = __float_as_uint(am);
                int e = (int)(bits >> 23) - 8 + ((bits & 0x7fffffu) > 0x600000u ? 1 : 0);
                e = e < 0 ? 0 : (e > 254 ? 254 : e);
                const float inv = __uint_as_float((uint32_t)(254 - e) << 23);
                uint32_t w[4];
#pragma unroll
                for (int h = 0; h < 4; ++h) {
                    int pk = __builtin_amdgcn_cvt_pk_fp8_f32(fminf(fmaxf(v[4 * h] * inv, -448.f), 448.f), fminf(fmaxf(v[4 * h + 1] * inv, -448.f), 448.f), 0, false);
                    pk = __builtin_amdgcn_cvt_pk_fp8_f32(fminf(fmaxf(v[4 * h + 2] * inv, -448.f), 448.f), fminf(fmaxf(v[4 * h + 3] * inv, -448.f), 448.f), pk, true);
                    w[h] = (uint32_t)pk;
                }
                st16(p.C8 + (int64_t)m * p.ldc8 + nb, make_uint4(w[0], w[1], w[2], w[3]));
                const int kb = nb >> 5;
                if ((g & 1) == 0) p.C8s[((int64_t)(kb >> 2) * p.M + m) * 4 + (kb & 3)] = (unsigned char)e;
            }
        }
    }
}

static inline int fast_epilogue_mask(const GemmP& p, bool out_f32) {
    auto al16 = [](const void* q) { return (reinterpret_cast<uintptr_t>(q) & 15) == 0; };
    const int esz = 2;
    if (p.c_mode != LNX_ADDR_PLAIN || p.cmap.group > 0 || p.cmap.off != 0 || p.gamma) return F_GENERIC;
    if (p.N % 16 != 0 || !al16(p.C) || (p.ldc * (out_f32 ? 4 : esz)) % 16 != 0) return F_GENERIC;
    const int64_t lim = (int64_t)1 << 31;
    if ((int64_t)p.M * p.ldc >= lim) return F_GENERIC;
    int f = 0;
    if (p.bias) {
        if (!al16(p.bias)) return F_GENERIC;
        f |= F_BIAS;
    }
    if (p.C2) {
        if (!al16(p.C2) || (p.ldc2 * esz) % 16 != 0 || (int64_t)p.M * p.ldc2 >= lim) return F_GENERIC;
        f |= F_C2;
    }
    if (p.act == LNX_ACT_GELU) f |= F_GELU;
    else if (p.act == LNX_ACT_GELU_D) {
        if (!p.C2) return F_GENERIC;
        f |= F_GELU;
    } else if (p.act == LNX_ACT_GELU_BWD || p.act == LNX_ACT_MUL_AUX) {
        if (!al16(p.aux) || (p.ldaux * esz) % 16 != 0 || (int64_t)p.M * p.ldaux >= lim) return F_GENERIC;
        f |= F_GELU_BWD;
    } else if (p.act != LNX_ACT_NONE) return F_GENERIC;
    if (p.res) {
        if (!al16(p.res) || (p.ldres * 4) % 16 != 0 || (int64_t)p.M * p.ldres >= lim) return F_GENERIC;
        f |= F_RES;
    }
    if (p.rowscale && !p.res) return F_GENERIC;
    if (!out_f32 && (f == 0 || f == F_BIAS || f == (F_BIAS | F_C2 | F_GELU) || f == (F_BIAS | F_GELU) || f == F_GELU_BWD)) return f;
    if (out_f32 && f == (F_BIAS | F_RES)) return f;
    return F_GENERIC;
}

struct WgradP {
    const unsigned char* dY;
    const unsigned char* A;
    float* dW;
    float* db;
    int64_t lddy, lda, lddw;
    int M, N, K;
    int a_mode;
    PatchGeom pg;
    int k_perm_c, k_store;
    float* ws;
    int64_t ws_floats;
    int tiles_n, tiles_k, splits, m_per_split;
};


struct NtSwitches {
    bool force_v1;
    bool skinny;
    bool v4;
    bool tile_cost;
    bool generic_epi;
    int v7, v9;
    bool fp8_x8;
};
NtSwitches nt_switches();

void fill_gemm_p(const lnx_gemm_args* a, GemmP& p);

struct NtChoice {
    int kind, f;
};
NtChoice nt_choose(const GemmP& p, int dtype, bool out_f32);

typedef int (*nt_experiment_fn)(const GemmP& p, int f, bool out_f32, hipStream_t st);
extern nt_experiment_fn g_nt_experiment;

void note_nt_kernel(int kind);

template <bool O, int FF>
struct NtForm {
    static constexpr bool out_f32 = O;
    static constexpr int f = FF;
};
int nt_form_error(const char* family, bool out_f32, int f);

template <auto Carries, bool O, int FF, class Launch>
int nt_form_case(const char* family, Launch& launch) {
    if constexpr (Carries(O, FF)) return launch(NtForm<O, FF>{});
    else return nt_form_error(family, O, FF);
}

template <auto Carries, class Launch>
int with_nt_form(const char* family, bool out_f32, int f, Launch&& launch) {
    if (f == F_GENERIC) return out_f32 ? nt_form_case<Carries, true, F_GENERIC>(family, launch) : nt_form_case<Carries, false, F_GENERIC>(family, launch);
    if (out_f32) {
        if (f == (F_BIAS | F_RES)) return nt_form_case<Carries, true, F_BIAS | F_RES>(family, launch);
        return nt_form_error(family, out_f32, f);
    }
    switch (f) {
        case 0: return nt_form_case<Carries, false, 0>(family, launch);
        case F_BIAS: return nt_form_case<Carries, false, F_BIAS>(family, launch);
        case F_BIAS | F_C2 | F_GELU: return nt_form_case<Carries, false, F_BIAS | F_C2 | F_GELU>(family, launch);
        case F_BIAS | F_C2 | F_GELU | F_MXOUT: return nt_form_case<Carries, false, F_BIAS | F_C2 | F_GELU | F_MXOUT>(family, launch);
        case F_BIAS | F_GELU: return nt_form_case<Carries, false, F_BIAS | F_GELU>(family, launch);
        case F_GELU_BWD: return nt_form_case<Carries, false, F_GELU_BWD>(family, launch);
        case F_GELU_BWD | F_MXOUT: return nt_form_case<Carries, false, F_GELU_BWD | F_MXOUT>(family, launch);
    }
    return nt_form_error(family, out_f32, f);
}

int launch_nt_v1(const GemmP& p, int dtype, bool out_f32, hipStream_t st);

bool nt_skinny_ok(const GemmP& p, int dtype, bool out_f32);
int launch_nt_skinny(const GemmP& p, bool out_f32, hipStream_t st);
int launch_nt_skinny_group(const GemmP* ps, int n, bool accumulate, bool out_f32, hipStream_t st);

constexpr int BM4 = 256, BN4 = 256, BK4 = 32, ROWB4 = 64;
int launch_nt_v2(const GemmP& p, int f, bool out_f32, hipStream_t st);
int launch_nt_v4(const GemmP& p, int f, bool out_f32, hipStream_t st);

bool nt_v7_ok(const GemmP& p, int f, bool out_f32);
int launch_nt_v7(const GemmP& p, int f, bool out_f32, hipStream_t st);

bool nt_v9_ok(const GemmP& p, int f, bool out_f32);
int launch_nt_v9(const GemmP& p, int f, bool out_f32, hipStream_t st);

int launch_tn_v2(const WgradP& p, int splits_hint, hipStream_t st, bool defer);
int tn_flush(hipStream_t st);
int tn_discard();
// ... 5 lines not shown
```

linnaeus_amd/csrc/gemm_nt_dispatch.cpp:

```cpp
#include <stdlib.h>

#include <atomic>

#include "gemm_common.hpp"

static std::atomic<int> g_last_nt{0};
static std::atomic<long long> g_nt_launches[LNX_NT_KERNEL_KINDS];
extern "C" int lnx_last_nt_kernel(void) { return g_last_nt.load(std::memory_order_relaxed); }
extern "C" int64_t lnx_nt_kernel_launches(int kind) {
    return (kind < 0 || kind >= LNX_NT_KERNEL_KINDS) ? -1 : (int64_t)g_nt_launches[kind].load(std::memory_order_relaxed);
}

namespace lnxg {

void note_nt_kernel(int kind) {
    if (kind < 0 || kind >= LNX_NT_KERNEL_KINDS) return;
    g_last_nt.store(kind, std::memory_order_relaxed);
    g_nt_launches[kind].fetch_add(1, std::memory_order_relaxed);
}

nt_experiment_fn g_nt_experiment = nullptr;

int nt_form_error(const char* family, bool out_f32, int f) {
    lnx_set_error("%s: no kernel is compiled for the epilogue form f = %d with %s output", family, f, out_f32 ? "an fp32" : "a storage-type");
    return 1;
}

static int env_int(const char* name, int unset) {
    const char* e = getenv(name);
    return e ? atoi(e) : unset;
}

NtSwitches nt_switches() {
    static const NtSwitches latched = [] {
        NtSwitches s{};
        s.force_v1 = getenv("LNX_GEMM_V1") != nullptr;
        s.skinny = env_int("LNX_NT_SKINNY", 1) != 0;
        s.v4 = env_int("LNX_NT_V4", 1) != 0;
        s.tile_cost = env_int("LNX_NT_TILE_COST", 1) != 0;
        s.generic_epi = getenv("LNX_NT_GENERIC_EPI") != nullptr;
        return s;
    }();
    NtSwitches s = latched;
    s.v7 = env_int("LNX_NT_V7", -1);
    s.v9 = env_int("LNX_NT_V9", -1);
    s.fp8_x8 = env_int("LNX_FP8_X8", 1) != 0;
    return s;
}

void fill_gemm_p(const lnx_gemm_args* a, GemmP& p) {
    p.A = (const unsigned char*)a->A;
    p.W = (const unsigned char*)a->W;
    p.C = (unsigned char*)a->C;
    p.C2 = (unsigned char*)a->c2;
    p.aux = (const unsigned char*)a->aux;
    p.bias = a->bias;
    p.gamma = a->gamma;
    p.rowscale = a->rowscale;
    p.res = a->res;
    p.lda = a->lda;
    p.ldw = a->ldw;
    p.ldc = a->ldc;
    p.ldc2 = a->ldc2;
    p.ldaux = a->ldaux;
    p.ldres = a->ldres;
    p.M = a->M;
    p.N = a->N;
    p.K = a->K;
    p.a_mode = a->a_mode;
    p.c_mode = a->c_mode;
    p.pg = PatchGeom{a->Hin, a->Win, a->Cin};
    p.cmap = RowMap{a->c_map.group, a->c_map.pad, a->c_map.off};
    p.act = a->act;
    p.rows_per_sample = a->rows_per_sample > 0 ? a->rows_per_sample : 1;
    p.tiles_m = cdiv(a->M, TILE);
    p.tiles_n = cdiv(a->N, TILE);
}

static bool big_tile_wins(const GemmP& p, const NtSwitches& sw) {
    if (!sw.tile_cost) return true;
    const int dc = device_cus();
    const int cus = persistent_cus(dc > 0 ? dc : 256);
    const int64_t rows = cdiv(p.M, 256);
    const double big = (double)cdiv(rows * (p.N / BN4), (int64_t)cus) * 2.0 * (p.K <= 512 ? 0.97 : 0.88);
    const double small = (double)cdiv(rows * cdiv(p.N, 128), (int64_t)cus);
    return small >= 0.93 * big;
}

static bool nt_v7_preferred(const GemmP& p, int f, bool out_f32, const NtSwitches& sw) {
    const bool two_per_cu = (int64_t)cdiv(p.M, 256) * cdiv(p.N, 128) >= 512;
    const bool big_better = p.N % BN4 == 0 && big_tile_wins(p, sw);
    if (f == F_GELU_BWD && p.act == LNX_ACT_MUL_AUX) return two_per_cu;
    if (f == F_GELU_BWD || f == (F_BIAS | F_C2 | F_GELU)) return two_per_cu && p.N % BN4 == 0 && !big_better;
    if (f != 0 && f != F_BIAS && !(out_f32 && f == (F_BIAS | F_RES))) return false;
    if (big_better) return false;
    return two_per_cu;
}

static bool nt_v4_ok(const GemmP& p, int f, const NtSwitches& sw) {
    if (!sw.v4 || f == (int)F_GENERIC || p.a_mode == LNX_ADDR_PATCH2) return false;
    return p.N % BN4 == 0 && p.K % BK4 == 0 && p.K >= 4 * BK4;
}

static bool nt_v2_ok(const GemmP& p, int dtype) {
    if (dtype != LNX_BF16) return false;
    if (p.K % 64 != 0 || p.K < 128) return false;
    if (p.M < 1024) return false;
    return true;
}

NtChoice nt_choose(const GemmP& p, int dtype, bool out_f32) {
    const NtSwitches sw = nt_switches();
    if (sw.skinny && !sw.force_v1 && nt_skinny_ok(p, dtype, out_f32)) return {LNX_NT_KERNEL_SKINNY, 0};
    if (sw.force_v1 || !nt_v2_ok(p, dtype)) return {LNX_NT_KERNEL_V1, 0};
    const int f = (p.a_mode == LNX_ADDR_PATCH2 || sw.generic_epi) ? (int)F_GENERIC : fast_epilogue_mask(p, out_f32);
    if (sw.v7 != 0 && nt_v7_ok(p, f, out_f32) && (sw.v7 == 1 || nt_v7_preferred(p, f, out_f32, sw))) return {LNX_NT_KERNEL_V7, f};
    if (nt_v4_ok(p, f, sw) && (sw.v9 == 1 || big_tile_wins(p, sw))) {
        const int dc = device_cus();
        const int64_t cus = dc > 0 ? dc : 256;
        if (sw.v9 != 0 && nt_v9_ok(p, f, out_f32) && (sw.v9 == 1 || (int64_t)cdiv(p.M, BM4) * (p.N / BN4) * 2 >= 3 * cus)) return {LNX_NT_KERNEL_V9, f};
        return {LNX_NT_KERNEL_V4, f};
    }
    return {LNX_NT_KERNEL_V2, f};
}

}

extern "C" int lnx_nt_dispatch(const lnx_gemm_args* a) {
    if (!a || a->M <= 0 || a->N <= 0 || a->K <= 0 || (a->dtype != LNX_F32 && a->dtype != LNX_BF16)) return -1;
    GemmP p;
    fill_gemm_p(a, p);
    return nt_choose(p, a->dtype, a->out_f32 != 0).kind;
}

extern "C" int lnx_gemm_nt(const lnx_gemm_args* a, void* stream) {
    LNX_CHECK(a != nullptr, "lnx_gemm_nt: null args");
    LNX_CHECK(a->dtype == LNX_F32 || a->dtype == LNX_BF16, "lnx_gemm_nt: bad dtype %d", a->dtype);
    const int epv = a->dtype == LNX_F32 ? 4 : 8;
    LNX_CHECK(a->M > 0 && a->N > 0 && a->K > 0, "lnx_gemm_nt: empty problem M=%d N=%d K=%d", a->M, a->N, a->K);
    LNX_CHECK(a->K % epv == 0, "lnx_gemm_nt: K=%d must be a multiple of %d", a->K, epv);
    LNX_CHECK(a->A && a->W && a->C, "lnx_gemm_nt: null operand");
    LNX_CHECK(a->ldw % epv == 0, "lnx_gemm_nt: ldw=%lld must be a multiple of %d", (long long)a->ldw, epv);
    LNX_CHECK((((uintptr_t)a->A) & 15) == 0 && (((uintptr_t)a->W) & 15) == 0, "lnx_gemm_nt: A/W must be 16-byte aligned");
    if (a->a_mode == LNX_ADDR_PATCH2) {
        LNX_CHECK(a->Hin % 2 == 0 && a->Win % 2 == 0 && a->Cin % epv == 0, "lnx_gemm_nt: bad PATCH2 geometry %dx%dx%d", a->Hin, a->Win, a->Cin);
        LNX_CHECK(a->K == 4 * a->Cin, "lnx_gemm_nt: PATCH2 needs K == 4*Cin");
        LNX_CHECK(a->M % ((a->Hin / 2) * (a->Win / 2)) == 0, "lnx_gemm_nt: PATCH2 needs M == B*Ho*Wo");
    } else {
        LNX_CHECK(a->lda % epv == 0, "lnx_gemm_nt: lda=%lld must be a multiple of %d", (long long)a->lda, epv);
    }
    if (a->c_mode == LNX_ADDR_PATCH2) {
        LNX_CHECK(a->Hin % 2 == 0 && a->Win % 2 == 0 && a->Cin % 16 == 0, "lnx_gemm_nt: bad PATCH2 output geometry");
        LNX_CHECK(a->N == 4 * a->Cin, "lnx_gemm_nt: PATCH2 output needs N == 4*Cin");
        LNX_CHECK(a->a_mode == LNX_ADDR_PLAIN, "lnx_gemm_nt: PATCH2 on both sides is not supported");
    }
    LNX_CHECK(a->act >= LNX_ACT_NONE && a->act <= LNX_ACT_MUL_AUX, "lnx_gemm_nt: unknown act %d", a->act);
    if (a->act == LNX_ACT_GELU_BWD || a->act == LNX_ACT_RELU_BWD || a->act == LNX_ACT_MUL_AUX) LNX_CHECK(a->aux != nullptr, "lnx_gemm_nt: act %d needs aux", a->act);
    if (a->act == LNX_ACT_GELU_D) LNX_CHECK(a->c2 != nullptr, "lnx_gemm_nt: GELU_D writes the derivative to c2, which is NULL");
    if (a->rowscale) LNX_CHECK(a->rows_per_sample > 0, "lnx_gemm_nt: rowscale needs rows_per_sample");

    GemmP p;
    fill_gemm_p(a, p);
    const bool out_f32 = a->out_f32 != 0;
    hipStream_t st = (hipStream_t)stream;
    const NtChoice c = nt_choose(p, a->dtype, out_f32);
// ... 21 lines not shown
```

linnaeus_amd/csrc/plan.cpp:

```cpp
#include <hip/hip_runtime.h>
#include <stdlib.h>
#include <string.h>

#include <mutex>
#include <atomic>
#include <string>
#include <vector>

#include "../../include/lnx.h"

void lnx_set_error(const char* fmt, ...);

#define RUN(expr)                  \
    do {                           \
        const int rc_ = (expr);    \
        if (rc_ != 0) return rc_;  \
    } while (0)
#define FAIL(...)                   \
    do {                            \
        lnx_set_error(__VA_ARGS__); \
        return 1;                   \
    } while (0)
#define HIPRUN(expr)                                                         \
    do {                                                                     \
// ... 71 lines not shown
    OpW stem_w, cl_w1, cl_w2;
    std::vector<int> head_b;
    std::vector<OpW> head_w;
    std::vector<int> logit_ld;
    std::vector<int64_t> logit_off;
    int64_t logits_numel = 0;
    Down down[3];
    std::vector<ConvBlk> conv[2];
    std::vector<RopeBlk> rope[2];
    std::vector<MetaHead> meta[2];
    std::vector<OpW*> all_w;
    std::vector<int> drop_conv[2], drop_attn[2], drop_mlp[2];
    int n_drop = 0;

    int64_t o_descs = 0, n_descs = 0, prep_blocks = 0;
    int64_t arena_end = 0;
    int64_t n_descs_t = 0, n_descs_f = 0, prep_blocks_f = 0;
    int64_t o_patches, o_stem_pre, o_stem_mean, o_stem_rstd;
    int64_t o_stage_out[4];
    int64_t o_tok[2];
    int64_t o_t1, o_t1_mean, o_t1_rstd;
    int64_t o_cl_hpre, o_cl_act, o_cl_u, o_cl_mean, o_cl_rstd, o_c1n;
    int64_t o_c2n, o_n2_mean, o_n2_rstd, o_agg, o_fin_mean, o_fin_rstd, o_feats, o_featsT;
    int64_t o_g[4];
    int64_t o_sA, o_sB = 0, o_sC, o_sD;
    int64_t o_lnws = 0, lnws_floats = 0, o_lnws_side = 0, lnws_side_floats = 0;
    int64_t lnws_defer_floats = 0;
    int64_t o_lnws_defer = 0;
    int ln_pending = 0;
    int64_t gcos_floats = 0;
    int freq_pending = 0;
    bool freq_defer = true;
    bool ln_defer = true;
    int64_t o_tnws = 0;
    int64_t o_lsws = 0, lsws_floats = 0;
    int64_t o_gcos , o_delta, o_dt1, o_tail[6], o_mtmp[4], o_dlT;
    int64_t o_a8 = 0, o_a8s = 0, o_h8 = 0, o_h8s = 0;
    const float* last_drop = nullptr;
    const unsigned char* last_mask = nullptr;
    std::vector<unsigned char> mask_host;
    const float* last_meta = nullptr;
    int resident[4] = {-1, -1, -1, -1};
    const unsigned char* dmask = nullptr;
    float inv_keep = 1.0f;
    int64_t dmask_bytes = 0;
    const unsigned char* amask = nullptr;
    float a_inv_keep = 1.0f;
    int64_t amask_bytes = 0;
    hipStream_t side = nullptr;
    hipEvent_t ev_fork = nullptr, ev_meta = nullptr, ev_bfork[2] = {nullptr, nullptr}, ev_bjoin[2] = {nullptr, nullptr};
    hipStream_t wgs = nullptr;
    bool wgs_on = true;
    bool meta_forked[2] = {false, false};
    int meta_mode = 1;
    bool meta_chain = true;
    bool chain_ok[2] = {false, false};
    bool dy8_ready = false;
    hipEvent_t ev_wf[4] = {nullptr, nullptr, nullptr, nullptr}, ev_wj[4] = {nullptr, nullptr, nullptr, nullptr};
    bool profile = false;
    bool profile_spans = false;
    struct Span { hipEvent_t e0, e1; int cls; double work, bytes; };
    std::vector<Span> spans;
    std::vector<hipEvent_t> ev_pool;
    size_t ev_used = 0;

    template <typename U> U* at(int64_t off) const { return reinterpret_cast<U*>(ws + off); }
// ... 168 lines not shown
}

extern "C" int lnx_plan_create(const lnx_mformer_cfg* cfg, lnx_plan** out) {
    if (!cfg || !out) FAIL("lnx_plan_create: null argument");
    const lnx_mformer_cfg& c = *cfg;
    if (c.dtype != LNX_F32 && c.dtype != LNX_BF16) FAIL("lnx_plan_create: bad dtype %d", c.dtype);
    if (c.batch <= 0 || c.img_h <= 0 || c.img_w <= 0 || c.in_chans <= 0 || c.in_chans > 4) FAIL("lnx_plan_create: bad input geometry");
    if (c.img_h % 32 != 0 || c.img_w % 32 != 0) FAIL("lnx_plan_create: image size %dx%d must be divisible by 32 (4*2*2*2 patchify)", c.img_h, c.img_w);
    for (int i = 0; i < 4; ++i)
        if (c.dims[i] <= 0 || c.dims[i] % 32 != 0 || c.dims[i] > 2048) FAIL("lnx_plan_create: dims[%d]=%d must be a multiple of 32 in (0, 2048]", i, c.dims[i]);
    for (int s = 0; s < 2; ++s) {
        if (c.conv_depths[s] < 0 || c.rope_depths[s] <= 0) FAIL("lnx_plan_create: bad depths");
        const int hd = c.rope_heads[s] > 0 && c.dims[2 + s] % c.rope_heads[s] == 0 ? c.dims[2 + s] / c.rope_heads[s] : 0;
        if (hd != 32 && hd != 64 && hd != 128)
            FAIL("lnx_plan_create: head_dim = dim / heads must be 32, 64 or 128 (dim %d, heads %d)", c.dims[2 + s], c.rope_heads[s]);
        if (c.mlp_hidden[s] <= 0 || c.mlp_hidden[s] % 16 != 0) FAIL("lnx_plan_create: mlp_hidden must be a multiple of 16");
    }
    if (c.n_meta < 0 || c.n_meta > LNX_MAX_META || c.n_tasks < 0 || c.n_tasks > LNX_MAX_TASKS) FAIL("lnx_plan_create: too many meta components / tasks");
    for (int m = 0; m < c.n_meta; ++m)
        if (c.meta_dims[m] <= 0 || c.meta_dims[m] > 16) FAIL("lnx_plan_create: meta dim %d must be in 1..16", c.meta_dims[m]);
    if (c.rope_mode != LNX_ROPE_COS && c.rope_mode != LNX_ROPE_ROTATE) FAIL("lnx_plan_create: rope_mode %d (LNX_ROPE_COS or LNX_ROPE_ROTATE)", c.rope_mode);

    if (c.fp8) {
        if (c.dtype != LNX_BF16) FAIL("lnx_plan_create: fp8 = 1 needs dtype = LNX_BF16 (fp8 operands, bf16 storage)");
        for (int s = 0; s < 2; ++s)
            if (c.dims[2 + s] % 128 != 0 || c.mlp_hidden[s] % 128 != 0)
                FAIL("lnx_plan_create: fp8 = 1 needs RoPE dims and MLP widths that are multiples of 128 (stage %d: %d / %d)", s + 2, c.dims[2 + s], c.mlp_hidden[s]);
    }
    lnx_plan* p = new lnx_plan();
    p->c = c;
    p->esz = c.dtype == LNX_BF16 ? 2 : 4;
    p->meta_chain = !env_off("LNX_META_CHAIN");
    p->ln_defer = !env_off("LNX_LN_DEFER");
    p->freq_defer = !env_off("LNX_FREQ_DEFER");
    for (int s = 0; s < 2; ++s) p->chain_ok[s] = p->meta_chain && lnx_meta_heads_supported(c.dims[2 + s]) != 0;
    p->E = 1 + c.n_meta;
    p->H[0] = c.img_h / 4;
    p->W[0] = c.img_w / 4;
    for (int i = 1; i < 4; ++i) {
        p->H[i] = p->H[i - 1] / 2;
        p->W[i] = p->W[i - 1] / 2;
    }
    for (int i = 0; i < 4; ++i) p->HW[i] = p->H[i] * p->W[i];
    for (int s = 0; s < 2; ++s) p->Ntok[s] = p->HW[2 + s] + p->E;
    build_params(p);
    const int* D = c.dims;
    const int B = c.batch;
    const int esz = p->esz;

    auto reg = [&](OpW& w) { p->all_w.push_back(&w); };
    reg(p->stem_w);
    for (int i = 0; i < 3; ++i) reg(p->down[i].w);
    for (int s = 0; s < 2; ++s)
        for (auto& k : p->conv[s]) {
            reg(k.w1);
            reg(k.w2);
        }
    for (int s = 0; s < 2; ++s)
        for (auto& k : p->rope[s]) {
            reg(k.qkv);
            reg(k.proj);
            reg(k.fc1);
            reg(k.fc2);
        }
    for (int s = 0; s < 2; ++s)
        for (auto& k : p->meta[s]) {
// ... 177 lines not shown
            if (M * D[2 + s] > mc) mc = M * D[2 + s];
            if (M * c.mlp_hidden[s] > mh) mh = M * c.mlp_hidden[s];
        }
        p->o_a8 = cv.take(mc);
        p->o_a8s = cv.take(mc / 32);
        p->o_h8 = cv.take(mh);
        p->o_h8s = cv.take(mh / 32);
    }
    if (!inf) {
        p->o_lnws = cv.take(p->lnws_floats * 4);
        {
            const int64_t rows[5] = {(int64_t)B * p->HW[0], (int64_t)B * p->HW[1], (int64_t)B * p->Ntok[0], (int64_t)B * p->Ntok[1], (int64_t)B};
            const int64_t wide[5] = {D[0], D[1], D[2], D[3], D[3]};
            int64_t need = 0;
            for (int i = 0; i < 5; ++i) {
                int64_t wgs = (rows[i] + 7) / 8;
                if (wgs > 2048) wgs = 2048;
                if (wgs * 2 * wide[i] > need) need = wgs * 2 * wide[i];
            }
            p->lnws_defer_floats = need;
            p->o_lnws_defer = cv.take(need * 4 * LN_DEFER_SLOTS);
        }
        p->o_lnws_side = cv.take(p->lnws_side_floats * 4);
        p->o_tnws = cv.take((int64_t)LNX_TN_WS_FLOATS * 4 * TN_WS_SLOTS);
        {
            const int64_t cmax = D[0] > D[1] ? D[0] : D[1];
            p->lsws_floats = cmax * 4 * cmax + cmax;
            p->o_lsws = cv.take(p->lsws_floats * 4);
        }
        p->o_sA = cv.take(maxM4C * esz);
        if (any_fused) p->o_sB = cv.take(maxM4C * esz);
        p->o_sC = cv.take(maxMC * esz);
        p->o_sD = cv.take(maxMC * esz);
    }
    if (!inf) {
        int64_t gmax = 0, dmax = 0;
        for (int s = 0; s < 2; ++s) {
            const int N = p->Ntok[s];
            const int64_t gsz = lnx_attn_bwd_ws_floats_hd(B, N, c.rope_heads[s], D[2 + s] / c.rope_heads[s]) * 4;
            const int64_t dsz = (int64_t)B * c.rope_heads[s] * N * 4;
            if (gsz > gmax) gmax = gsz;
            if (dsz > dmax) dmax = dsz;
        }
        p->gcos_floats = gmax / 4;
        p->o_gcos = cv.take(gmax * FREQ_DEFER_SLOTS);
        p->o_delta = cv.take(dmax);
    }
    for (int s = 0; s < 2; ++s) {
        const int64_t N = p->Ntok[s], M = B * N, C = D[2 + s], hid = c.mlp_hidden[s];
        for (auto& k : p->rope[s]) {
            k.dm_proj = p->dmask_bytes;
            k.dm_hid = k.dm_proj + M * C;
            k.dm_fc2 = k.dm_hid + M * hid;
            p->dmask_bytes = k.dm_fc2 + M * C;
            k.dm_attn = p->amask_bytes;
            p->amask_bytes += (int64_t)B * c.rope_heads[s] * N * ((N + 63) / 64 * 64);
        }
    }
    p->ws_bytes = cv.cur;
    *out = p;
    return 0;
}

extern "C" int64_t lnx_plan_dropout_bytes(const lnx_plan* p) { return p ? p->dmask_bytes : 0; }
extern "C" int64_t lnx_plan_attn_dropout_bytes(const lnx_plan* p) { return p ? p->amask_bytes : 0; }

// ... 839 lines not shown
        ++p->freq_pending;
    }
    ab.dsin_tab = c.at<float>(k.dsin); ab.dfreqs = p->G[k.freqs];
    if (p->c.rope_mode == LNX_ROPE_ROTATE) {
        ab.rope_mode = LNX_ROPE_ROTATE; ab.sin_tab = c.at<float>(k.dsin); ab.dsin_tab = nullptr; ab.grid_w = p->W[2 + s];
    }
    if (p->amask) {
        ab.drop_mask = p->amask + k.dm_attn; ab.drop_inv_keep = p->a_inv_keep;
    }
    {
        Timed t(c, 3, 14.0 * B * (double)N * N * C);
        RUN(lnx_attn_bwd(&ab, c.st));
    }
    RUN(wfork(3));
    RUN(wgrad(cw, M, 3 * C, C, sA, 3 * C, c.at<void>(k.n1), C, k.qkv.param, k.qkvb, C, 0, 3));
    RUN(lnx_gemm_tn_flush(cw.st));
    RUN(wdone(3));
    RUN(wjoin(2));
    a = gemm_base(c, M, C, 3 * C, sA, 3 * C, c.wtptr(k.qkv), k.qkv.ld_t, sC, C, false);
    RUN(gemm_nt_t(c, &a));
    Dx2 d1;
    if (i > 0) {
        d1.p = sC; d1.rowscale = p->drop_ptr(p->drop_mlp[s][i - 1]); d1.rps = N;
        if (mx_dgrad) {
            d1.p8 = c.at<void>(p->o_a8); d1.p8s = c.at<void>(p->o_a8s);
            p->dy8_ready = true;
        }
    }
    RUN(ln_bwd(c, M, C, sC, c.dt, C, IDM, c.at<float>(k.xin), LNX_F32, C, IDM, k.n1w, k.n1b, c.at<float>(k.mean1), c.at<float>(k.rstd1), g, g, LNX_F32, C, false, d1));
    RUN(wjoin(3));
    return 0;
}

int conv_block_bwd(const Ctx& c, int s, int i, float* g) {
    lnx_plan* p = c.p;
    ConvBlk& k = p->conv[s][i];
    const int B = p->c.batch, H = p->H[s], W = p->W[s], C = p->c.dims[s];
    const int M = B * H * W;
    void* sA = c.at<void>(p->o_sA);
    void* sC = c.at<void>(p->o_sC);
    void* sD = c.at<void>(p->o_sD);
    Timed span(c, 9, 4.0 * M * C * (8.0 * C + 49.0));
    bool forked = false, joined = false;
    if (k.fused) {
        void* sB = c.at<void>(p->o_sB);
        lnx_convmlp_bwd_args f;
        memset(&f, 0, sizeof f);
        f.dtype = c.dt; f.M = M; f.C = C;
        f.g = g; f.ln = c.at<void>(k.ln); f.w1 = c.wptr(k.w1); f.b1 = p->P[k.b1];
        f.w2t = c.wtptr(k.w2); f.w1t = c.wtptr(k.w1); f.gamma = p->P[k.gamma];
        f.rowscale = p->drop_ptr(p->drop_conv[s][i]); f.rows_per_sample = H * W;
        f.act = sB; f.dh = sA; f.dz = sC; f.dln = sD; f.dgamma = p->G[k.gamma];
        f.dz_plain = 1;
        if (k.fused_ln) {
            f.y = c.at<void>(k.y); f.ln_w = p->P[k.lnw]; f.mean = c.at<float>(k.mean); f.rstd = c.at<float>(k.rstd);
            f.d_ln_w = p->G[k.lnw]; f.d_ln_b = p->G[k.lnb];
            f.ws = c.at<float>(p->o_lnws); f.ws_floats = p->lnws_floats;
            if (p->ln_defer && p->o_lnws_defer != 0 && lnx_convmlp_bwd_ws_floats(C, M) <= p->lnws_defer_floats) {
                RUN(ln_defer_slot(c, f.ws, f.ws_floats));
                f.ln_defer = 1;
            }
        }
        {
            Timed t(c, 7, 2.0 * M * C * 4 * C * 3);
            RUN(lnx_convmlp_bwd(&f, c.st));
        }
        const Ctx cw = wg_ctx(c);
        RUN(wg_fork(c, 0));
        forked = true;
        float* S = c.at<float>(p->o_lsws);
        float* T = S + (int64_t)C * 4 * C;
        HIPRUN(hipMemsetAsync(S, 0, ((size_t)C * 4 * C + C) * 4, (hipStream_t)cw.st));
        RUN(wgrad_into(cw, M, C, 4 * C, sC, C, sB, 4 * C, S, T, 4 * C, 0));
        RUN(wgrad(cw, M, 4 * C, C, sA, 4 * C, c.at<void>(k.ln), C, k.w1.param, k.b1, C, 0, 1));
        RUN(lnx_gemm_tn_flush(cw.st));
        RUN(lnx_layerscale_apply_wgrad(S, T, 4 * C, p->P[k.w2.param], p->P[k.b2], 4 * C, p->P[k.gamma], p->G[k.w2.param], p->G[k.b2], 4 * C, p->G[k.gamma], C, 4 * C, cw.st));
        RUN(wg_done(c, 0));
        if (!k.fused_ln) {
            RUN(wg_join(c, 0));
            joined = true;
        }
    } else {
        RUN(lnx_layerscale_bwd(g, c.at<void>(k.z), c.dt, p->P[k.gamma], p->drop_ptr(p->drop_conv[s][i]), H * W, sC, p->G[k.gamma], M, C, c.st));
        RUN(wgrad(c, M, C, 4 * C, sC, C, c.at<void>(k.act), 4 * C, k.w2.param, k.b2, 4 * C));
        lnx_gemm_args a = gemm_base(c, M, 4 * C, C, sC, C, c.wtptr(k.w2), k.w2.ld_t, sA, 4 * C, false);
        a.act = LNX_ACT_MUL_AUX; a.aux = c.at<void>(k.hpre); a.ldaux = 4 * C;
        RUN(gemm_nt_t(c, &a));
        RUN(wgrad(c, M, 4 * C, C, sA, 4 * C, c.at<void>(k.ln), C, k.w1.param, k.b1, C));
        a = gemm_base(c, M, C, 4 * C, sA, 4 * C, c.wtptr(k.w1), k.w1.ld_t, sD, C, false);
        RUN(gemm_nt_t(c, &a));
    }
    void* dy = sD;
    if (!k.fused_ln) {
        RUN(ln_bwd(c, M, C, sD, c.dt, C, IDM, c.at<void>(k.y), c.dt, C, IDM, k.lnw, k.lnb, c.at<float>(k.mean), c.at<float>(k.rstd), nullptr, sC, c.dt, C, false));
        dy = sC;
    }
    lnx_dwconv_wgrad_args w;
    memset(&w, 0, sizeof w);
    w.B = B; w.H = H; w.W = W; w.C = C;
    w.x = c.at<float>(k.xin); w.x_dtype = LNX_F32; w.dy = dy; w.dy_dtype = c.dt;
    w.dw = p->G[k.dww]; w.db = p->G[k.dwb];
    {
        Timed t(c, 5, (double)M * C * (4 + p->esz));
        RUN(lnx_dwconv7_wgrad(&w, c.st));
    }
    lnx_dwconv_args d;
    memset(&d, 0, sizeof d);
    d.B = B; d.H = H; d.W = W; d.C = C;
    d.x = dy; d.x_dtype = c.dt; d.w49 = c.at<float>(k.w49); d.bias = nullptr; d.flip = 1; d.res = g; d.y = g; d.y_dtype = LNX_F32;
    {
        Timed t(c, 4, (double)M * C * (8 + p->esz));
        RUN(lnx_dwconv7_fwd(&d, c.st));
    }
    if (forked && !joined) RUN(wg_join(c, 0));
    return 0;
}

int downsample_bwd(const Ctx& c, int i, const float* gout, int64_t ldg, lnx_rowmap gmap, const void* x, int xdt, int64_t ldx, lnx_rowmap xm, void* dx, int dxdt,
                   int64_t lddx) {
    lnx_plan* p = c.p;
    Down& d = p->down[i];
    const int B = p->c.batch, Hin = p->H[i], Win = p->W[i], Cin = p->c.dims[i], Cout = p->c.dims[i + 1];
    const int Min = B * Hin * Win, Mout = Min / 4;
    void* sA = c.at<void>(p->o_sA);
    void* sC = c.at<void>(p->o_sC);
    RUN(lnx_scale_cast(gout, ldg, gmap, nullptr, 0, sC, c.dt, Cout, Mout, Cout, c.st));
    lnx_wgrad_args w;
    memset(&w, 0, sizeof w);
    w.dtype = c.dt; w.M = Mout; w.N = Cout; w.K = 4 * Cin;
    w.dY = sC; w.lddy = Cout; w.A = c.at<void>(d.ln); w.a_mode = LNX_ADDR_PATCH2; w.Hin = Hin; w.Win = Win; w.Cin = Cin;
    w.dW = p->G[d.w.param]; w.lddw = 4 * Cin; w.k_perm_c = Cin; w.db = p->G[d.cb];
    w.ws = c.at<float>(p->o_tnws); w.ws_floats = LNX_TN_WS_FLOATS;
    {
        Timed t(c, 1, 2.0 * Mout * Cout * 4 * Cin);
        RUN(lnx_gemm_tn(&w, c.st));
    }
    lnx_gemm_args a = gemm_base(c, Mout, 4 * Cin, Cout, sC, Cout, c.wtptr(d.w), d.w.ld_t, sA, 0, false);
    a.c_mode = LNX_ADDR_PATCH2; a.Hin = Hin; a.Win = Win; a.Cin = Cin;
    RUN(gemm_nt_t(c, &a));
    RUN(ln_bwd(c, Min, Cin, sA, c.dt, Cin, IDM, x, xdt, ldx, xm, d.lnw, d.lnb, c.at<float>(d.mean), c.at<float>(d.rstd), nullptr, dx, dxdt, lddx, false));
    return 0;
}

int meta_head_bwd(const Ctx& cc, int s, int m, const float* g) {
    const Ctx c{cc.p, cc.st, LNX_F32};
    lnx_plan* p = c.p;
    MetaHead& k = p->meta[s][m];
    const int B = p->c.batch, C = p->c.dims[2 + s], N = p->Ntok[s];
    float* dtok = c.at<float>(p->o_mtmp[0]);
    void* t1 = c.at<void>(p->o_mtmp[1]);
    void* t2 = c.at<void>(p->o_mtmp[2]);
    float* dxf = c.at<float>(p->o_mtmp[3]);
    const lnx_rowmap rm = {1, N - 1, 1 + m};
    RUN(lnx_scale_cast(g, C, rm, nullptr, 0, dtok, LNX_F32, C, B, C, c.st));
    RUN(ln_bwd(c, B, C, dtok, LNX_F32, C, IDM, c.at<void>(k.h2), c.dt, C, IDM, k.nf2w, k.nf2b, c.at<float>(k.m2), c.at<float>(k.r2), nullptr, t1, c.dt, C, true));
    RUN(wgrad(c, B, C, C, t1, C, c.at<void>(k.n1), C, k.w2.param, k.b2, C));
    lnx_gemm_args a = gemm_base(c, B, C, C, t1, C, c.wtptr(k.w2), k.w2.ld_t, t2, C, false);
    RUN(gemm_nt_t(c, &a));
    RUN(ln_bwd(c, B, C, t2, c.dt, C, IDM, c.at<void>(k.h1), c.dt, C, IDM, k.nf1w, k.nf1b, c.at<float>(k.m1), c.at<float>(k.r1), nullptr, t1, c.dt, C, true));
    RUN(wgrad(c, B, C, C, t1, C, c.at<void>(k.x), C, k.w1.param, k.b1, C));
    a = gemm_base(c, B, C, C, t1, C, c.wtptr(k.w1), k.w1.ld_t, dxf, C, true);
    a.res = dtok; a.ldres = C;
    RUN(gemm_nt_t(c, &a));
    RUN(ln_bwd(c, B, C, dxf, LNX_F32, C, IDM, c.at<void>(k.h0), c.dt, C, IDM, k.lnw0, k.lnb0, c.at<float>(k.m0), c.at<float>(k.r0), nullptr, t1, c.dt, C, true));
    RUN(wgrad(c, B, C, 16, t1, C, c.at<void>(k.t0), 16, k.w0.param, k.b0, k.dim, k.dim));
    return 0;
}

int meta_bwd(const Ctx& c, int s, const float* g) {
    if (c.p->chain_ok[s]) return meta_chain_bwd(c, s, g);
// ... 145 lines not shown
            RUN(ln_bwd(c, B, C, dc1n, LNX_F32, C, IDM, c.at<float>(p->o_cl_u), LNX_F32, C, IDM, p->cl_lnw, p->cl_lnb, c.at<float>(p->o_cl_mean), c.at<float>(p->o_cl_rstd),
                       nullptr, du, cf.dtype, C, false));
            RUN(wgrad(c, B, C, C2, du, C, c.at<void>(p->o_cl_act), C2, p->cl_w2.param, p->cl_b2, C2));
            lnx_gemm_args a = gemm_base(c, B, C2, C, du, C, c.wtptr(p->cl_w2), p->cl_w2.ld_t, dca, C2, false);
            a.act = LNX_ACT_GELU_BWD; a.aux = c.at<void>(p->o_cl_hpre); a.ldaux = C2;
            RUN(gemm_nt_t(c, &a));
            RUN(wgrad(c, B, C2, C2, dca, C2, c.at<void>(p->o_t1), (int64_t)p->Ntok[0] * C2, p->cl_w1.param, p->cl_b1, C2));
            a = gemm_base(c, B, C2, C2, dca, C2, c.wtptr(p->cl_w1), p->cl_w1.ld_t, dt1, C2, false);
            a.c_map = lnx_rowmap{1, p->Ntok[0] - 1, 0};
            RUN(gemm_nt_t(c, &a));
        }
        float* g2 = c.at<float>(p->o_g[2]);
        Dx2 dn;
        dn.p = c.at<void>(p->o_sC); dn.rowscale = p->drop_ptr(p->drop_mlp[0][cf.rope_depths[0] - 1]); dn.rps = p->Ntok[0];
        RUN(ln_bwd(c, B * p->Ntok[0], C2, dt1, cf.dtype, C2, IDM, c.at<float>(p->o_stage_out[2]), LNX_F32, C2, IDM, p->norm_w[0], p->norm_b[0], c.at<float>(p->o_t1_mean),
                   c.at<float>(p->o_t1_rstd), nullptr, g2, LNX_F32, C2, false, dn));
        RUN(ln_flush(c));
        if (heads_forked) RUN(wg_join(c, 3));
    }
    if (all || segment == 1) {
        float* g2 = c.at<float>(p->o_g[2]);
        for (int i = cf.rope_depths[0] - 1; i >= 0; --i) {
            RUN(rope_block_restore(c, 0, i));
            RUN(rope_block_bwd(c, 0, i, g2, true));
        }
        RUN(tokens_bwd(c, 0, g2));
        const lnx_rowmap gm = {p->HW[2], p->E, p->E};
        RUN(downsample_bwd(c, 1, g2, D[2], gm, c.at<float>(p->o_stage_out[1]), LNX_F32, D[1], IDM, c.at<float>(p->o_g[1]), LNX_F32, D[1]));
        RUN(ln_flush(c));
        RUN(join_side(c, 1));
    }
    if (all || segment == 2) {
        float* g1 = c.at<float>(p->o_g[1]);
        for (int i = cf.conv_depths[1] - 1; i >= 0; --i) {
            RUN(conv_block_restore(c, 1, i));
            RUN(conv_block_bwd(c, 1, i, g1));
        }
        RUN(downsample_bwd(c, 0, g1, D[1], IDM, c.at<float>(p->o_stage_out[0]), LNX_F32, D[0], IDM, c.at<float>(p->o_g[0]), LNX_F32, D[0]));
        RUN(ln_flush(c));
        RUN(join_side(c, 0));
    }
    if (all || segment == 3) {
        float* g0 = c.at<float>(p->o_g[0]);
        for (int i = cf.conv_depths[0] - 1; i >= 0; --i) {
            RUN(conv_block_restore(c, 0, i));
            RUN(conv_block_bwd(c, 0, i, g0));
        }
        const int M0 = B * p->HW[0];
        void* sC = c.at<void>(p->o_sC);
        RUN(ln_bwd(c, M0, D[0], g0, LNX_F32, D[0], IDM, c.at<void>(p->o_stem_pre), cf.dtype, D[0], IDM, p->stem_lnw, p->stem_lnb, c.at<float>(p->o_stem_mean),
                   c.at<float>(p->o_stem_rstd), nullptr, sC, cf.dtype, D[0], false));
        const int kst = cf.in_chans * 16;
        RUN(wgrad(c, M0, D[0], 64, sC, D[0], c.at<void>(p->o_patches), 64, p->stem_w.param, p->stem_b, kst, kst));
        RUN(ln_flush(c));
    }
    return 0;
}

extern "C" int lnx_plan_backward_into(lnx_plan* p, const float* dlogits, const float* dfeats, float* const* grads, void* stream) {
    if (!p || !grads) FAIL("lnx_plan_backward_into: null %s", !p ? "plan" : "gradient pointer set");
    if (!p->bound || !p->has_grads) FAIL("lnx_plan_backward_into: plan is not bound with gradient buffers");
    const size_t n = p->names.size();
    for (size_t i = 0; i < n; ++i)
        if (grads[i] == nullptr || (((uintptr_t)grads[i]) & 3) != 0) FAIL("lnx_plan_backward_into: gradient of %s is null or misaligned", p->names[i].c_str());
    std::vector<float*> into(grads, grads + n);
    struct Swap {
        lnx_plan* p;
        std::vector<float*>& v;
        Swap(lnx_plan* p_, std::vector<float*>& v_) : p(p_), v(v_) { p->G.swap(v); }
        ~Swap() { p->G.swap(v); }
    } swap{p, into};
// ... 81 lines not shown
```

linnaeus_amd/ops.py:

```python
from __future__ import annotations

import ctypes as C
from typing import Optional, Tuple

import torch

from . import _lib as L
from ._lib import F32, BF16

_TORCH_DT = {F32: torch.float32, BF16: torch.bfloat16}


def code_of(t: torch.Tensor) -> int:
    if t.dtype == torch.float32:
        return F32
    if t.dtype == torch.bfloat16:
        return BF16
    raise L.LnxError(f"unsupported tensor dtype {t.dtype}")


def torch_dtype(code: int) -> torch.dtype:
    return _TORCH_DT[code]


# ... 172 lines not shown
    a.dy, a.dy_dtype, a.lddy, a.dy_map = _p(dy), code_of(dy), (lddy if lddy is not None else dy.stride(-2)), _map(dy_map)
    a.x, a.x_dtype, a.ldx, a.x_map = _p(x), code_of(x), (ldx if ldx is not None else x.stride(-2)), _map(x_map)
    a.w, a.mean, a.rstd = _p(w), _p(mean), _p(rstd)
    a.gin, a.ldgin = _p(gin), ((ldgin if ldgin is not None else gin.stride(-2)) if gin is not None else 0)
    a.dx, a.dx_dtype, a.lddx = _p(dx), code_of(dx), (lddx if lddx is not None else dx.stride(-2))
    a.dw, a.db, a.relu_mask = _p(dw), _p(db), int(relu_mask)
    a.ws, a.ws_floats = _p(ws), (ws.numel() if ws is not None else 0)
    a.defer = int(defer)
    if dx2 is not None:
        a.dx2, a.dx2_dtype, a.lddx2 = _p(dx2), code_of(dx2), (lddx2 if lddx2 is not None else dx2.stride(-2))
        a.dx2_rowscale, a.dx2_rows_per_sample = _p(dx2_rowscale), int(dx2_rows_per_sample)
        if dx2_8 is not None:
            a.dx2_8, a.dx2_8_scales, a.lddx2_8 = _p(dx2_8), _p(dx2_8_scales), dx2_8.stride(-2)
    return a


def layernorm_bwd(dy, x, w, mean, rstd, dx, **kw):
    a = _ln_bwd_args(dy, x, w, mean, rstd, dx, **kw)
    L.check(L.lib().lnx_layernorm_bwd(C.byref(a), _stream()), "lnx_layernorm_bwd")
    return dx


def layernorm_bwd_query(dy, x, w, mean, rstd, dx, **kw) -> L.LnLaunch:
    a, out = _ln_bwd_args(dy, x, w, mean, rstd, dx, **kw), L.LnLaunch()
    if L.lib().lnx_layernorm_bwd_query(C.byref(a), C.byref(out)) != 0:
        raise L.LnxError(f"lnx_layernorm_bwd_query refused: {L.lib().lnx_last_error().decode()}")
    return out


def layernorm_bwd_flush():
    L.check(L.lib().lnx_layernorm_bwd_flush(_stream()), "lnx_layernorm_bwd_flush")


def dwconv7(x, w49, bias, y, *, flip=False, res=None):
    B, H, W, Cc = x.shape
    a = L.DwconvArgs()
    a.B, a.H, a.W, a.C = B, H, W, Cc
    a.x, a.x_dtype, a.w49, a.bias = _p(x), code_of(x), _p(w49), _p(bias)
    a.flip, a.res, a.y, a.y_dtype = int(flip), _p(res), _p(y), code_of(y)
    L.check(L.lib().lnx_dwconv7_fwd(C.byref(a), _stream()), "lnx_dwconv7_fwd")
    return y


def dwconv7_wgrad(x, dy, dw, db):
    B, H, W, Cc = x.shape
    a = L.DwconvWgradArgs()
    a.B, a.H, a.W, a.C = B, H, W, Cc
    a.x, a.x_dtype, a.dy, a.dy_dtype, a.dw, a.db = _p(x), code_of(x), _p(dy), code_of(dy), _p(dw), _p(db)
    L.check(L.lib().lnx_dwconv7_wgrad(C.byref(a), _stream()), "lnx_dwconv7_wgrad")


def rope_cos_table(freqs, H, W, out=None, dsin=None):
    heads, half = freqs.shape[1], freqs.shape[2]
    if out is None:
        out = torch.empty(H * W, heads, half, device=freqs.device, dtype=torch.float32)
    L.check(L.lib().lnx_rope_cos_table_hd(_p(freqs), heads, 2 * half, H, W, _p(out), _p(dsin) if dsin is not None else None, _stream()),
            "lnx_rope_cos_table_hd")
    return out


def rope_cossin_table(freqs, H, W):
    heads, half = freqs.shape[1], freqs.shape[2]
    cos = torch.empty(H * W, heads, half, device=freqs.device, dtype=torch.float32)
    sin = torch.empty_like(cos)
    L.check(L.lib().lnx_rope_cossin_table_hd(_p(freqs), heads, 2 * half, H, W, _p(cos), _p(sin), None, _stream()), "lnx_rope_cossin_table_hd")
    return cos, sin


def rope_cos_tables(entries):
    arr = (L.RopeTable * len(entries))()
    for t, (freqs, H, W, out, dsin, *rest) in zip(arr, entries):
        t.freqs, t.cos_out, t.dsin_out = _p(freqs), _p(out), _p(dsin) if dsin is not None else None
# ... 82 lines not shown
    L.check(L.lib().lnx_colsum_rows(_p(inp), C.c_int64(ldin), _map(row_map), _p(out), M, Cc, _stream()), "lnx_colsum_rows")


def agg2_fwd(a, b, w2, bias1, out, M, Cc):
    L.check(L.lib().lnx_agg2_fwd(_p(a), _p(b), _p(w2), _p(bias1), _p(out), M, Cc, _stream()), "lnx_agg2_fwd")


def agg2_bwd(dout, a, b, w2, da, db, dw2, dbias1, M, Cc):
    L.check(L.lib().lnx_agg2_bwd(_p(dout), _p(a), _p(b), _p(w2), _p(da), _p(db), _p(dw2), _p(dbias1), M, Cc, _stream()), "lnx_agg2_bwd")


def pack_meta(meta, off, dim, out):
    L.check(L.lib().lnx_pack_meta(_p(meta), meta.shape[1], off, dim, _p(out), code_of(out), meta.shape[0], _stream()), "lnx_pack_meta")


def convmlp_fwd(ln, w1, b1, w2, b2, gamma, x, out, *, rowscale=None, rows_per_sample=0, z=None, y=None, ln_w=None, ln_b=None, ln_eps=1e-6,
                ln_out=None, mean=None, rstd=None):
    a = L.ConvMlpArgs()
    src = ln if y is None else y
    a.dtype, a.M, a.C = code_of(src), src.shape[0], src.shape[1]
    a.ln, a.w1, a.b1, a.w2, a.b2, a.gamma = _p(ln), _p(w1), _p(b1), _p(w2), _p(b2), _p(gamma)
    a.rowscale, a.rows_per_sample, a.x, a.out, a.z = _p(rowscale), rows_per_sample, _p(x), _p(out), _p(z)
    a.y, a.ln_w, a.ln_b, a.ln_eps, a.ln_out, a.mean, a.rstd = _p(y), _p(ln_w), _p(ln_b), ln_eps, _p(ln_out), _p(mean), _p(rstd)
    L.check(L.lib().lnx_convmlp_fwd(C.byref(a), _stream()), "lnx_convmlp_fwd")
    return out


def layerscale_apply_wgrad(s, t, w, b, gamma, dw, db, dgamma):
    L.check(L.lib().lnx_layerscale_apply_wgrad(_p(s), _p(t), C.c_int64(s.stride(0)), _p(w), _p(b), C.c_int64(w.stride(0)), _p(gamma), _p(dw), _p(db),
                                               C.c_int64(dw.stride(0)), _p(dgamma), w.shape[0], w.shape[1], _stream()), "lnx_layerscale_apply_wgrad")


def convmlp_bwd(g, ln, z, w1, b1, w2t, w1t, gamma, act, dh, dz, dln, dgamma, *, rowscale=None, rows_per_sample=0, y=None, ln_w=None, mean=None,
                rstd=None, d_ln_w=None, d_ln_b=None, ws=None, dz_plain=False):
    a = L.ConvMlpBwdArgs()
    a.dtype, a.M, a.C = code_of(ln), ln.shape[0], ln.shape[1]
    a.g, a.ln, a.z, a.w1, a.b1, a.w2t, a.w1t, a.gamma = _p(g), _p(ln), _p(z), _p(w1), _p(b1), _p(w2t), _p(w1t), _p(gamma)
    a.rowscale, a.rows_per_sample = _p(rowscale), rows_per_sample
    a.act, a.dh, a.dz, a.dln, a.dgamma = _p(act), _p(dh), _p(dz), _p(dln), _p(dgamma)
    a.y, a.ln_w, a.mean, a.rstd, a.d_ln_w, a.d_ln_b = _p(y), _p(ln_w), _p(mean), _p(rstd), _p(d_ln_w), _p(d_ln_b)
    a.ws, a.ws_floats = _p(ws), (ws.numel() if ws is not None else 0)
    a.dz_plain = int(dz_plain)
    L.check(L.lib().lnx_convmlp_bwd(C.byref(a), _stream()), "lnx_convmlp_bwd")


def _meta_head_buffers(B, C_, dev):
    f = lambda *shape: torch.empty(*shape, device=dev, dtype=torch.float32)
    return {"t0": f(B, 16), "h0": f(B, C_), "x": f(B, C_), "h1": f(B, C_), "n1": f(B, C_), "h2": f(B, C_),
            "m0": f(B), "r0": f(B), "m1": f(B), "r1": f(B), "m2": f(B), "r2": f(B)}


def meta_heads_fwd(meta, heads, tok, eps=1e-5):
    B = meta.shape[0]
    arr = (L.MetaHeadArgs * len(heads))()
    keep, saved = [], []
    for i, h in enumerate(heads):
        C_ = h["w1"].shape[0]
        w0p = torch.zeros(C_, 16, device=meta.device)
        w0p[:, :h["dim"]] = h["w0"]
        bufs = _meta_head_buffers(B, C_, meta.device)
        t = tok[i] if isinstance(tok, (list, tuple)) else tok
        a = arr[i]
        a.B, a.C, a.dim, a.off, a.meta, a.meta_width, a.eps = B, C_, h["dim"], h["off"], _p(meta), meta.shape[1], eps
        a.w0, a.ldw0, a.b0, a.ln0_w, a.ln0_b = _p(w0p), 16, _p(h["b0"]), _p(h["ln0_w"]), _p(h["ln0_b"])
        a.w1, a.ldw1, a.b1, a.ln1_w, a.ln1_b = _p(h["w1"]), C_, _p(h["b1"]), _p(h["ln1_w"]), _p(h["ln1_b"])
        a.w2, a.ldw2, a.b2, a.ln2_w, a.ln2_b = _p(h["w2"]), C_, _p(h["b2"]), _p(h["ln2_w"]), _p(h["ln2_b"])
        for k_, v in bufs.items():
            setattr(a, k_, _p(v))
        a.tok, a.tok_row_stride, a.tok_row_offset = _p(t), t.shape[1] * C_, h["slot"] * C_
        keep.append(w0p)
        saved.append(bufs)
    L.check(L.lib().lnx_meta_heads_fwd(arr, len(heads), _stream()), "lnx_meta_heads_fwd")
    return saved


# ... 121 lines not shown
```

Measured before the change: 13710 images/sec.

## Recompute LN output from y in convmlp bwd and emit bf16 grad copy from dwconv

The convmlp backward kernel can now rebuild the LayerNorm output from the pre-norm input y using the saved mean/rstd and ln_b, instead of reading a stored ln tensor. The dwconv backward launch can write a bf16 copy of the fp32 gradient in its epilogue, which lets downsample_bwd skip a separate scale_cast pass. The GEMM v2 path also now accepts the plain and bias-only epilogues. Together these are meant to cut memory traffic and kernel launches in the stage-1 backward pass, at the cost of extra ALU work, a little more LDS and a reused scratch region.

Result: no change. 13690 images/sec, median of 2 (-0.1%).

```diff
diff --git a/include/lnx.h b/include/lnx.h
--- a/include/lnx.h
+++ b/include/lnx.h
@@ -65,6 +65,8 @@
 int lnx_last_nt_kernel(void);
 int64_t lnx_nt_kernel_launches(int kind);
 int lnx_nt_dispatch(const lnx_gemm_args* args);
+enum { LNX_NT_EPILOGUE_GENERIC = 1 << 10 };
+int lnx_nt_dispatch_epilogue(const lnx_gemm_args* args);
 
 int lnx_amax(const void* x, int x_dtype, int64_t ldx, int rows, int cols, float* amax, void* stream);
 int lnx_quantize_fp8(const void* x, int x_dtype, int64_t ldx, int rows, int cols, const float* amax, void* y, int64_t ldy, float* scale_out, void* stream);
@@ -183,6 +185,7 @@
     const float* res;
     void* y;
     int y_dtype;
+    void* y16;
 } lnx_dwconv_args;
 int lnx_dwconv7_fwd(const lnx_dwconv_args* args, void* stream);
 
@@ -697,6 +700,7 @@
     int64_t ws_floats;
     int dz_plain;
     int ln_defer;
+    const float* ln_b;
 } lnx_convmlp_bwd_args;
 int lnx_convmlp_bwd(const lnx_convmlp_bwd_args* args, void* stream);
 int64_t lnx_convmlp_bwd_ws_floats(int C, int M);
diff --git a/linnaeus_amd/_lib.py b/linnaeus_amd/_lib.py
--- a/linnaeus_amd/_lib.py
+++ b/linnaeus_amd/_lib.py
@@ -255,7 +255,7 @@
 
 EXPORTS = [
     "lnx_last_error", "lnx_version", "lnx_device_cus", "lnx_set_cu_margin",
-    "lnx_gemm_nt", "lnx_last_nt_kernel", "lnx_nt_kernel_launches", "lnx_nt_dispatch", "lnx_gemm_tn", "lnx_gemm_tn_flush", "lnx_gemm_tn_discard", "lnx_amax", "lnx_quantize_fp8", "lnx_gemm_nt_fp8", "lnx_quantize_mxfp8", "lnx_gemm_nt_mxfp8", "lnx_dropout_mul", "lnx_dropout_residual", "lnx_plan_dropout_bytes", "lnx_plan_set_dropout", "lnx_plan_attn_dropout_bytes", "lnx_plan_set_attn_dropout",
+    "lnx_gemm_nt", "lnx_last_nt_kernel", "lnx_nt_kernel_launches", "lnx_nt_dispatch", "lnx_nt_dispatch_epilogue", "lnx_gemm_tn", "lnx_gemm_tn_flush", "lnx_gemm_tn_discard", "lnx_amax", "lnx_quantize_fp8", "lnx_gemm_nt_fp8", "lnx_quantize_mxfp8", "lnx_gemm_nt_mxfp8", "lnx_dropout_mul", "lnx_dropout_residual", "lnx_plan_dropout_bytes", "lnx_plan_set_dropout", "lnx_plan_attn_dropout_bytes", "lnx_plan_set_attn_dropout",
     "lnx_layernorm_fwd", "lnx_layernorm_bwd", "lnx_layernorm_bwd_flush", "lnx_layernorm_bwd_discard", "lnx_layernorm_fwd_query", "lnx_layernorm_bwd_query",
     "lnx_dwconv7_fwd", "lnx_dwconv7_wgrad",
     "lnx_gemm_nt_group_ok", "lnx_gemm_nt_group", "lnx_rope_cos_table", "lnx_rope_cos_table_hd", "lnx_rope_cossin_table_hd", "lnx_rope_cos_tables", "lnx_attn_bwd_ws_floats", "lnx_attn_bwd_ws_floats_hd", "lnx_attn_fwd", "lnx_attn_bwd", "lnx_attn_bwd_flush", "lnx_attn_bwd_discard", "lnx_attn_dispatch", "lnx_last_attn_kernel", "lnx_last_attn_bwd_launches",
@@ -346,7 +346,7 @@
     _fields_ = [
         ("B", C.c_int), ("H", C.c_int), ("W", C.c_int), ("C", C.c_int),
         ("x", C.c_void_p), ("x_dtype", C.c_int), ("w49", C.c_void_p), ("bias", C.c_void_p),
-        ("flip", C.c_int), ("res", C.c_void_p), ("y", C.c_void_p), ("y_dtype", C.c_int),
+        ("flip", C.c_int), ("res", C.c_void_p), ("y", C.c_void_p), ("y_dtype", C.c_int), ("y16", C.c_void_p),
     ]
 
 
@@ -408,7 +408,7 @@
         ("act", C.c_void_p), ("dh", C.c_void_p), ("dz", C.c_void_p), ("dln", C.c_void_p), ("dgamma", C.c_void_p),
         ("y", C.c_void_p), ("ln_w", C.c_void_p), ("mean", C.c_void_p), ("rstd", C.c_void_p), ("d_ln_w", C.c_void_p), ("d_ln_b", C.c_void_p),
         ("ws", C.c_void_p), ("ws_floats", C.c_int64),
-        ("dz_plain", C.c_int), ("ln_defer", C.c_int),
+        ("dz_plain", C.c_int), ("ln_defer", C.c_int), ("ln_b", C.c_void_p),
     ]
 
 
diff --git a/linnaeus_amd/csrc/api.cpp b/linnaeus_amd/csrc/api.cpp
--- a/linnaeus_amd/csrc/api.cpp
+++ b/linnaeus_amd/csrc/api.cpp
@@ -19,7 +19,7 @@
 }
 
 extern "C" const char* lnx_last_error(void) { return g_err; }
-extern "C" int lnx_version(void) { return 109; }
+extern "C" int lnx_version(void) { return 110; }
 extern "C" int lnx_device_cus(void) {
     int dev = 0;
     if (hipGetDevice(&dev) != hipSuccess) return -1;
diff --git a/linnaeus_amd/csrc/convmlp.hip b/linnaeus_amd/csrc/convmlp.hip
--- a/linnaeus_amd/csrc/convmlp.hip
+++ b/linnaeus_amd/csrc/convmlp.hip
@@ -263,28 +263,7 @@
     return v;
 }
 template <int NK>
-__device__ __forceinline__ void ln_row_frags(uint4 (&xf)[NK], const float* w, const float* b, int g, float eps, float& mu, float& rs) {
-    constexpr float invC = 1.0f / (float)Geo<NK>::C;
-    float v[NK][8];
-    float sum = 0.f;
-#pragma unroll
-    for (int ks = 0; ks < NK; ++ks) {
-        Vec16<bf16_t> t;
-        t.raw = xf[ks];
-#pragma unroll
-        for (int j = 0; j < 8; ++j) v[ks][j] = t.get(j);
-        sum += ((v[ks][0] + v[ks][1]) + (v[ks][2] + v[ks][3])) + ((v[ks][4] + v[ks][5]) + (v[ks][6] + v[ks][7]));
-    }
-    mu = g_sum(sum) * invC;
-    float sq = 0.f;
-#pragma unroll
-    for (int ks = 0; ks < NK; ++ks)
-#pragma unroll
-        for (int j = 0; j < 8; ++j) {
-            v[ks][j] -= mu;
-            sq = fmaf(v[ks][j], v[ks][j], sq);
-        }
-    rs = 1.0f / sqrtf(fmaf(g_sum(sq), invC, eps));
+__device__ __forceinline__ void ln_apply_frags(uint4 (&xf)[NK], const float* w, const float* b, int g, float mu, float rs) {
 #pragma unroll
     for (int ks = 0; ks < NK; ++ks) {
         const int c = ks * 32 + 8 * g;
@@ -292,11 +271,37 @@
         const float4 b0 = *reinterpret_cast<const float4*>(b + c), b1 = *reinterpret_cast<const float4*>(b + c + 4);
         const float wv[8] = {w0.x, w0.y, w0.z, w0.w, w1.x, w1.y, w1.z, w1.w};
         const float bv[8] = {b0.x, b0.y, b0.z, b0.w, b1.x, b1.y, b1.z, b1.w};
-        Vec16<bf16_t> o;
-#pragma unroll
-        for (int j = 0; j < 8; ++j) o.set(j, fmaf(v[ks][j] * rs, wv[j], bv[j]));
+        Vec16<bf16_t> t, o;
+        t.raw = xf[ks];
+#pragma unroll
+        for (int j = 0; j < 8; ++j) o.set(j, fmaf((t.get(j) - mu) * rs, wv[j], bv[j]));
         xf[ks] = o.raw;
     }
+}
+template <int NK>
+__device__ __forceinline__ void ln_row_frags(uint4 (&xf)[NK], const float* w, const float* b, int g, float eps, float& mu, float& rs) {
+    constexpr float invC = 1.0f / (float)Geo<NK>::C;
+    float v[NK][8];
+    float sum = 0.f;
+#pragma unroll
+    for (int ks = 0; ks < NK; ++ks) {
+        Vec16<bf16_t> t;
+        t.raw = xf[ks];
+#pragma unroll
+        for (int j = 0; j < 8; ++j) v[ks][j] = t.get(j);
+        sum += ((v[ks][0] + v[ks][1]) + (v[ks][2] + v[ks][3])) + ((v[ks][4] + v[ks][5]) + (v[ks][6] + v[ks][7]));
+    }
+    mu = g_sum(sum) * invC;
+    float sq = 0.f;
+#pragma unroll
+    for (int ks = 0; ks < NK; ++ks)
+#pragma unroll
+        for (int j = 0; j < 8; ++j) {
+            v[ks][j] -= mu;
+            sq = fmaf(v[ks][j], v[ks][j], sq);
+        }
+    rs = 1.0f / sqrtf(fmaf(g_sum(sq), invC, eps));
+    ln_apply_frags<NK>(xf, w, b, g, mu, rs);
 }
 template <int NK>
 struct LnRow {
@@ -523,6 +528,8 @@
     float* dgs = b1s + 4 * C;
     float* lws = dgs + C;
     float* dls = lws + C;
+    float* lbs = dls + 2 * C;
+    const bool ln_from_y = LNB && p.ln == nullptr;
 
     const int lane = threadIdx.x & 63;
     const int wave = __builtin_amdgcn_readfirstlane(threadIdx.x >> 6);
@@ -536,12 +543,16 @@
         if constexpr (LNB) {
             lws[i] = p.lnw[i];
             dls[i] = dls[C + i] = 0.f;
+            lbs[i] = ln_from_y ? p.lnb[i] : 0.f;
         }
     }
     __syncthreads();
 
     uint4 xf[MT][NK], zf[MT][NK];
     bool mvalid[MT];
+    const unsigned char* const xsrc = ln_from_y ? p.y : p.ln;
+    LnRow<NK> lrow;
+    if constexpr (LNB) ln_bwd_fetch<NK>(lrow, p, m_base + s, g);
 #pragma unroll
     for (int mt = 0; mt < MT; ++mt) {
         int m = m_base + mt * 16 + s;
@@ -553,7 +564,7 @@
 #pragma unroll
         for (int ks = 0; ks < NK; ++ks) {
             const int c = ks * 32 + 8 * g;
-            xf[mt][ks] = ld16(p.ln + ((int64_t)m * C + c) * 2);
+            xf[mt][ks] = ld16(xsrc + ((int64_t)m * C + c) * 2);
             g0v[ks] = *reinterpret_cast<const float4*>(p.g + (int64_t)m * C + c);
             g1v[ks] = *reinterpret_cast<const float4*>(p.g + (int64_t)m * C + c + 4);
             a0v[ks] = *reinterpret_cast<const float4*>(p.gamma + c);
@@ -586,14 +597,14 @@
             zf[mt][ks] = dzv.raw;
             st16(p.dz + ((int64_t)m * C + c) * 2, dzs.raw);
         }
+        if constexpr (LNB)
+            if (ln_from_y) ln_apply_frags<NK>(xf[mt], lws, lbs, g, lrow.mu, lrow.rs);
     }
     f32x4_t dl[CT][MT];
 #pragma unroll
     for (int ct = 0; ct < CT; ++ct)
 #pragma unroll
         for (int mt = 0; mt < MT; ++mt) dl[ct][mt] = f32x4_t{0.f, 0.f, 0.f, 0.f};
-    LnRow<NK> lrow;
-    if constexpr (LNB) ln_bwd_fetch<NK>(lrow, p, m_base + s, g);
 
     __syncthreads();
     dma_nmajor<NK, NW>(smem, p.w1, 0, wave, lane);
@@ -1213,7 +1224,7 @@
 
 template <int NK, int MT, int NW, bool ST, bool LNB, bool DG>
 int launch_bwd_t(const CmP& p, hipStream_t st) {
-    const size_t lds = 2 * 3 * Geo<NK>::PART + 8 * Geo<NK>::C * sizeof(float);
+    const size_t lds = 2 * 3 * Geo<NK>::PART + 9 * Geo<NK>::C * sizeof(float);
     static bool attr = false;
     if (!attr) {
         (void)hipFuncSetAttribute(reinterpret_cast<const void*>(&convmlp_bwd_kernel<NK, MT, NW, ST, LNB, DG>), hipFuncAttributeMaxDynamicSharedMemorySize, (int)lds);
@@ -1272,15 +1283,15 @@
 }
 
 extern "C" int lnx_convmlp_bwd(const lnx_convmlp_bwd_args* a, void* stream) {
-    LNX_CHECK(a && a->g && a->ln && a->w1 && a->w2t && a->w1t && a->b1 && a->gamma && a->dz && a->dln && (a->dgamma || !a->z),
-              "lnx_convmlp_bwd: null operand (z may be NULL: dgamma is then not produced here; with z, dgamma is required)");
+    LNX_CHECK(a && a->g && (a->ln || (a->y && a->ln_b && a->C > 96)) && a->w1 && a->w2t && a->w1t && a->b1 && a->gamma && a->dz && a->dln && (a->dgamma || !a->z),
+              "lnx_convmlp_bwd: null operand (z may be NULL: dgamma is then not produced here; with z, dgamma is required; ln may be NULL with y and ln_b in the streamed-weight kernels, C > 96)");
     LNX_CHECK((a->act == nullptr) == (a->dh == nullptr), "lnx_convmlp_bwd: act and dh must both be given or both be NULL");
     LNX_CHECK(lnx_convmlp_supported(a->dtype, a->C), "lnx_convmlp_bwd: unsupported dtype %d / C %d", a->dtype, a->C);
     LNX_CHECK(a->M > 0, "lnx_convmlp_bwd: empty");
     if (a->rowscale) LNX_CHECK(a->rows_per_sample > 0, "lnx_convmlp_bwd: rowscale needs rows_per_sample");
     if (a->y) LNX_CHECK(a->ln_w && a->mean && a->rstd && a->d_ln_w && a->d_ln_b && a->ws, "lnx_convmlp_bwd: the fused LayerNorm form needs ln_w, mean, rstd, d_ln_w, d_ln_b and ws");
     CmP p{};
-    p.y = (const unsigned char*)a->y; p.lnw = a->ln_w; p.mean = const_cast<float*>(a->mean); p.rstd = const_cast<float*>(a->rstd);
+    p.y = (const unsigned char*)a->y; p.lnw = a->ln_w; p.lnb = a->ln_b; p.mean = const_cast<float*>(a->mean); p.rstd = const_cast<float*>(a->rstd);
     p.part = a->ws; p.part_floats = a->ws_floats; p.dlnw = a->d_ln_w; p.dlnb = a->d_ln_b; p.ln_defer = a->ln_defer;
     p.g = a->g; p.ln = (const unsigned char*)a->ln; p.zin = (const unsigned char*)a->z; p.w1 = (const unsigned char*)a->w1;
     p.w2t = (const unsigned char*)a->w2t; p.w1t = (const unsigned char*)a->w1t; p.b1 = a->b1; p.gamma = a->gamma; p.rowscale = a->rowscale;
diff --git a/linnaeus_amd/csrc/dwconv.hip b/linnaeus_amd/csrc/dwconv.hip
--- a/linnaeus_amd/csrc/dwconv.hip
+++ b/linnaeus_amd/csrc/dwconv.hip
@@ -281,6 +281,7 @@
 extern "C" int lnx_dwconv7_fwd(const lnx_dwconv_args* a, void* stream) {
     LNX_CHECK(a && a->x && a->w49 && a->y, "lnx_dwconv7_fwd: null operand");
     LNX_CHECK(a->B > 0 && a->H > 0 && a->W > 0 && a->C > 0 && a->C % CB == 0, "lnx_dwconv7_fwd: bad shape B=%d H=%d W=%d C=%d (C %% 32)", a->B, a->H, a->W, a->C);
+    if (a->y16) LNX_CHECK(a->x_dtype == LNX_BF16 && a->y_dtype == LNX_F32, "lnx_dwconv7_fwd: y16 needs a bf16 x and an fp32 y");
     if (lnx_dwconv_mfma_enabled() && (a->x_dtype == LNX_BF16 || a->y_dtype == LNX_BF16) && !(a->res && a->y_dtype != LNX_F32))
         return lnx_dwconv7_mfma_fwd(a, (hipStream_t)stream);
     DwP p;
@@ -309,6 +310,10 @@
     }
 #undef DWL
     LNX_LAUNCH_CHECK();
+    if (a->y16) {
+        const lnx_rowmap idm = {0, 0, 0};
+        return lnx_scale_cast(static_cast<const float*>(a->y), a->C, idm, nullptr, 0, a->y16, LNX_BF16, a->C, (int)((int64_t)a->B * a->H * a->W), a->C, stream);
+    }
     return 0;
 }
 
diff --git a/linnaeus_amd/csrc/dwconv_mfma.hip b/linnaeus_amd/csrc/dwconv_mfma.hip
--- a/linnaeus_amd/csrc/dwconv_mfma.hip
+++ b/linnaeus_amd/csrc/dwconv_mfma.hip
@@ -20,6 +20,10 @@
 }
 __device__ __forceinline__ void buf_st16(__amdgpu_buffer_rsrc_t r, u32 voff, uint4 v) {
     __builtin_amdgcn_raw_buffer_store_b128(u32x4{v.x, v.y, v.z, v.w}, r, voff, 0, 0);
+}
+__device__ __forceinline__ void buf_st8(__amdgpu_buffer_rsrc_t r, u32 voff, uint2 v) {
+    typedef __attribute__((ext_vector_type(2))) u32 u32x2;
+    __builtin_amdgcn_raw_buffer_store_b64(u32x2{v.x, v.y}, r, voff, 0, 0);
 }
 constexpr int CPW = 2;
 
@@ -161,6 +165,7 @@
     const float* bias;
     const float* res;
     void* y;
+    void* y16;
     int B, H, W, C;
     int tiles_h, tiles_w, tiles_per_wg, ntile, chunks;
 };
@@ -199,8 +204,9 @@
 #define DWM_T(i) do { } while (0)
 #endif
 
-template <typename TX, typename TY, bool FLIP>
+template <typename TX, typename TY, bool FLIP, bool Y16 = false>
 __global__ __launch_bounds__(FT) void dwconv7_mfma_kernel(const MfP p) {
+    static_assert(!Y16 || sizeof(TY) == 4, "the bf16 copy goes with an fp32 output");
     extern __shared__ __attribute__((aligned(16))) char smem[];
     typedef Stage<TX, FT, FCB, MI, MI / 2, XPITCH, XPLANE> St;
     typedef OutT<TY> Ot;
@@ -334,6 +340,7 @@
         DWM_T(3);
         {
             const __amdgpu_buffer_rsrc_t yr = tile_rsrc(reinterpret_cast<const TY*>(p.y) + tile0);
+            const __amdgpu_buffer_rsrc_t yr16 = tile_rsrc(reinterpret_cast<const bf16_t*>(Y16 ? p.y16 : p.y) + tile0);
 #pragma unroll
             for (int k = 0; k < Ot::NPO; ++k) {
                 const char* o = ot + ol[k];
@@ -351,6 +358,7 @@
                         v.z += __builtin_bit_cast(float, rv[k].z); v.w += __builtin_bit_cast(float, rv[k].w);
                     }
                     buf_st16(yr, go[k], make_uint4(__builtin_bit_cast(u32, v.x), __builtin_bit_cast(u32, v.y), __builtin_bit_cast(u32, v.z), __builtin_bit_cast(u32, v.w)));
+                    if constexpr (Y16) buf_st8(yr16, go[k] == OOB ? OOB : go[k] >> 1, make_uint2(pack2(v.x, v.y), pack2(v.z, v.w)));
                 }
             }
         }
@@ -499,14 +507,14 @@
     return 0;
 }
 
-template <typename TX, typename TY, bool FLIP> int launch_fwd(const MfP& p, int grid, hipStream_t st) {
+template <typename TX, typename TY, bool FLIP, bool Y16 = false> int launch_fwd(const MfP& p, int grid, hipStream_t st) {
     const int lds = X_BYTES + OutT<TY>::BYTES;
     static bool ready = false;
     if (!ready) {
-        if (int rc = set_lds(dwconv7_mfma_kernel<TX, TY, FLIP>, lds)) return rc;
+        if (int rc = set_lds(dwconv7_mfma_kernel<TX, TY, FLIP, Y16>, lds)) return rc;
         ready = true;
     }
-    hipLaunchKernelGGL((dwconv7_mfma_kernel<TX, TY, FLIP>), dim3(grid), dim3(FT), lds, st, p);
+    hipLaunchKernelGGL((dwconv7_mfma_kernel<TX, TY, FLIP, Y16>), dim3(grid), dim3(FT), lds, st, p);
     return 0;
 }
 
@@ -535,7 +543,7 @@
 
 int lnx_dwconv7_mfma_fwd(const lnx_dwconv_args* a, hipStream_t st) {
     MfP p;
-    p.x = a->x; p.w49 = a->w49; p.bias = a->bias; p.res = a->res; p.y = a->y;
+    p.x = a->x; p.w49 = a->w49; p.bias = a->bias; p.res = a->res; p.y = a->y; p.y16 = a->y16;
     p.B = a->B; p.H = a->H; p.W = a->W; p.C = a->C;
     const int code = a->x_dtype * 2 + a->y_dtype + (a->flip ? 4 : 0);
     p.tiles_h = cdiv(a->H, MT); p.tiles_w = cdiv(a->W, MT);
@@ -553,10 +561,10 @@
     int rc = 0;
     switch (code) {
         case 1: rc = launch_fwd<float, bf16_t, false>(p, grid, st); break;
-        case 2: rc = launch_fwd<bf16_t, float, false>(p, grid, st); break;
+        case 2: rc = a->y16 ? launch_fwd<bf16_t, float, false, true>(p, grid, st) : launch_fwd<bf16_t, float, false>(p, grid, st); break;
         case 3: rc = launch_fwd<bf16_t, bf16_t, false>(p, grid, st); break;
         case 5: rc = launch_fwd<float, bf16_t, true>(p, grid, st); break;
-        case 6: rc = launch_fwd<bf16_t, float, true>(p, grid, st); break;
+        case 6: rc = a->y16 ? launch_fwd<bf16_t, float, true, true>(p, grid, st) : launch_fwd<bf16_t, float, true>(p, grid, st); break;
         case 7: rc = launch_fwd<bf16_t, bf16_t, true>(p, grid, st); break;
         default: LNX_CHECK(false, "lnx_dwconv7_fwd: the MFMA path needs a bf16 operand");
     }
diff --git a/linnaeus_amd/csrc/gemm2.hip b/linnaeus_amd/csrc/gemm2.hip
--- a/linnaeus_amd/csrc/gemm2.hip
+++ b/linnaeus_amd/csrc/gemm2.hip
@@ -254,7 +254,7 @@
     if (out_f32) return f == (F_BIAS | F_RES);
     return f == 0 || f == F_BIAS || f == (F_BIAS | F_C2 | F_GELU) || f == (F_BIAS | F_GELU) || f == F_GELU_BWD;
 }
-constexpr bool nt_v2_carries(bool out_f32, int f) { return f == F_GENERIC || nt_v4_carries(out_f32, f); }
+constexpr bool nt_v2_carries(bool out_f32, int f) { return f == F_GENERIC || f == 0 || f == F_BIAS || nt_v4_carries(out_f32, f); }
 
 int launch_nt_v4(const GemmP& p0, int f, bool out_f32, hipStream_t st) {
     GemmP p = p0;
@@ -274,10 +274,10 @@
     const int grid = p.tiles_m * p.tiles_n;
     const size_t lds = NSTAGE * STAGE_BYTES;
     const bool patch = p.a_mode == LNX_ADDR_PATCH2;
-    LNX_CHECK(!patch || f == F_GENERIC, "gemm_nt_v2: the 2x2 patch gather is compiled with the generic epilogue only (f = %d)", f);
+    LNX_CHECK(!patch || f == F_GENERIC || f == 0 || f == F_BIAS, "gemm_nt_v2: the 2x2 patch gather is compiled with the generic, plain and bias epilogues only (f = %d)", f);
     return with_nt_form<nt_v2_carries>("gemm_nt_v2", out_f32, f, [&](auto form) {
         using Form = decltype(form);
-        if constexpr (Form::f == F_GENERIC) {
+        if constexpr (Form::f == F_GENERIC || Form::f == 0 || Form::f == F_BIAS) {
             if (patch) return launch_with_lds<gemm_nt_v2_kernel<Form::out_f32, true, Form::f>>(grid, 512, lds, st, p);
         }
         return launch_with_lds<gemm_nt_v2_kernel<Form::out_f32, false, Form::f>>(grid, 512, lds, st, p);
diff --git a/linnaeus_amd/csrc/gemm3.hip b/linnaeus_amd/csrc/gemm3.hip
--- a/linnaeus_amd/csrc/gemm3.hip
+++ b/linnaeus_amd/csrc/gemm3.hip
@@ -362,7 +362,7 @@
 }
 
 bool nt_v7_ok(const GemmP& p, int f, bool out_f32) {
-    if (p.a_mode == LNX_ADDR_PATCH2) return false;
+    if (p.a_mode == LNX_ADDR_PATCH2 || p.c_mode != LNX_ADDR_PLAIN) return false;
     if (p.act == LNX_ACT_GELU_D) return false;
     if (p.K % BK7 != 0 || p.K / BK7 < 6) return false;
     if (p.N % 64 != 0) return false;
diff --git a/linnaeus_amd/csrc/gemm5.hip b/linnaeus_amd/csrc/gemm5.hip
--- a/linnaeus_amd/csrc/gemm5.hip
+++ b/linnaeus_amd/csrc/gemm5.hip
@@ -220,7 +220,7 @@
 }
 
 bool nt_v9_ok(const GemmP& p, int f, bool out_f32) {
-    if (p.a_mode == LNX_ADDR_PATCH2) return false;
+    if (p.a_mode == LNX_ADDR_PATCH2 || p.c_mode != LNX_ADDR_PLAIN) return false;
     if (p.N % BN9 != 0 || p.K % BK9 != 0 || p.K / BK9 < 8) return false;
     const int64_t lim = (int64_t)1 << 31;
     if ((int64_t)p.M * p.lda * 2 >= lim || (int64_t)p.N * p.ldw * 2 >= lim) return false;
diff --git a/linnaeus_amd/csrc/gemm_common.hpp b/linnaeus_amd/csrc/gemm_common.hpp
--- a/linnaeus_amd/csrc/gemm_common.hpp
+++ b/linnaeus_amd/csrc/gemm_common.hpp
@@ -328,7 +328,9 @@
 #pragma unroll
             for (int j = 0; j < 16; ++j) v[j] = fmaf(v[j], rs[mi], ld[mi][j]);
         }
-        const int coff = m * (int)p.ldc + nb;
+        int coff = m * (int)p.ldc + nb;
+        if constexpr (F == 0 || F == F_BIAS)
+            if (p.c_mode == LNX_ADDR_PATCH2) coff = (int)(patch_base(p.pg, m) + patch_col(p.pg, nb));
         if (OUT_F32) {
             float* cp = reinterpret_cast<float*>(p.C) + coff;
 #pragma unroll
@@ -370,13 +372,15 @@
     }
 }
 
-static inline int fast_epilogue_mask(const GemmP& p, bool out_f32) {
+static inline int fast_epilogue_mask(const GemmP& p, bool out_f32, bool patch_fast = true) {
     auto al16 = [](const void* q) { return (reinterpret_cast<uintptr_t>(q) & 15) == 0; };
     const int esz = 2;
-    if (p.c_mode != LNX_ADDR_PLAIN || p.cmap.group > 0 || p.cmap.off != 0 || p.gamma) return F_GENERIC;
-    if (p.N % 16 != 0 || !al16(p.C) || (p.ldc * (out_f32 ? 4 : esz)) % 16 != 0) return F_GENERIC;
+    const bool patch_c = p.c_mode == LNX_ADDR_PATCH2;
+    if ((patch_c && !patch_fast) || p.cmap.group > 0 || p.cmap.off != 0 || p.gamma) return F_GENERIC;
+    if (patch_c && (p.C2 || p.res || p.rowscale || p.act != LNX_ACT_NONE)) return F_GENERIC;
+    if (p.N % 16 != 0 || !al16(p.C) || (!patch_c && (p.ldc * (out_f32 ? 4 : esz)) % 16 != 0)) return F_GENERIC;
     const int64_t lim = (int64_t)1 << 31;
-    if ((int64_t)p.M * p.ldc >= lim) return F_GENERIC;
+    if ((int64_t)p.M * (patch_c ? (int64_t)p.N : p.ldc) >= lim) return F_GENERIC;
     int f = 0;
     if (p.bias) {
         if (!al16(p.bias)) return F_GENERIC;
@@ -401,6 +405,7 @@
     if (p.rowscale && !p.res) return F_GENERIC;
     if (!out_f32 && (f == 0 || f == F_BIAS || f == (F_BIAS | F_C2 | F_GELU) || f == (F_BIAS | F_GELU) || f == F_GELU_BWD)) return f;
     if (out_f32 && f == (F_BIAS | F_RES)) return f;
+    if (out_f32 && patch_fast && (f == 0 || f == F_BIAS) && (patch_c || p.a_mode == LNX_ADDR_PATCH2)) return f;
     return F_GENERIC;
 }
 
@@ -426,6 +431,7 @@
     bool v4;
     bool tile_cost;
     bool generic_epi;
+    bool patch_fast;
     int v7, v9;
     bool fp8_x8;
 };
@@ -461,6 +467,8 @@
     if (f == F_GENERIC) return out_f32 ? nt_form_case<Carries, true, F_GENERIC>(family, launch) : nt_form_case<Carries, false, F_GENERIC>(family, launch);
     if (out_f32) {
         if (f == (F_BIAS | F_RES)) return nt_form_case<Carries, true, F_BIAS | F_RES>(family, launch);
+        if (f == 0) return nt_form_case<Carries, true, 0>(family, launch);
+        if (f == F_BIAS) return nt_form_case<Carries, true, F_BIAS>(family, launch);
         return nt_form_error(family, out_f32, f);
     }
     switch (f) {
diff --git a/linnaeus_amd/csrc/gemm_nt_dispatch.cpp b/linnaeus_amd/csrc/gemm_nt_dispatch.cpp
--- a/linnaeus_amd/csrc/gemm_nt_dispatch.cpp
+++ b/linnaeus_amd/csrc/gemm_nt_dispatch.cpp
@@ -45,6 +45,7 @@
     s.v7 = env_int("LNX_NT_V7", -1);
     s.v9 = env_int("LNX_NT_V9", -1);
     s.fp8_x8 = env_int("LNX_FP8_X8", 1) != 0;
+    s.patch_fast = env_int("LNX_NT_PATCH_FAST", 1) != 0;
     return s;
 }
 
@@ -98,7 +99,7 @@
 }
 
 static bool nt_v4_ok(const GemmP& p, int f, const NtSwitches& sw) {
-    if (!sw.v4 || f == (int)F_GENERIC || p.a_mode == LNX_ADDR_PATCH2) return false;
+    if (!sw.v4 || f == (int)F_GENERIC || p.a_mode == LNX_ADDR_PATCH2 || p.c_mode != LNX_ADDR_PLAIN) return false;
     return p.N % BN4 == 0 && p.K % BK4 == 0 && p.K >= 4 * BK4;
 }
 
@@ -113,7 +114,7 @@
     const NtSwitches sw = nt_switches();
     if (sw.skinny && !sw.force_v1 && nt_skinny_ok(p, dtype, out_f32)) return {LNX_NT_KERNEL_SKINNY, 0};
     if (sw.force_v1 || !nt_v2_ok(p, dtype)) return {LNX_NT_KERNEL_V1, 0};
-    const int f = (p.a_mode == LNX_ADDR_PATCH2 || sw.generic_epi) ? (int)F_GENERIC : fast_epilogue_mask(p, out_f32);
+    const int f = ((p.a_mode == LNX_ADDR_PATCH2 && !sw.patch_fast) || sw.generic_epi) ? (int)F_GENERIC : fast_epilogue_mask(p, out_f32, sw.patch_fast);
     if (sw.v7 != 0 && nt_v7_ok(p, f, out_f32) && (sw.v7 == 1 || nt_v7_preferred(p, f, out_f32, sw))) return {LNX_NT_KERNEL_V7, f};
     if (nt_v4_ok(p, f, sw) && (sw.v9 == 1 || big_tile_wins(p, sw))) {
         const int dc = device_cus();
@@ -131,6 +132,14 @@
     GemmP p;
     fill_gemm_p(a, p);
     return nt_choose(p, a->dtype, a->out_f32 != 0).kind;
+}
+
+extern "C" int lnx_nt_dispatch_epilogue(const lnx_gemm_args* a) {
+    static_assert((int)LNX_NT_EPILOGUE_GENERIC == (int)F_GENERIC, "include/lnx.h names the generic epilogue's mask");
+    if (!a || a->M <= 0 || a->N <= 0 || a->K <= 0 || (a->dtype != LNX_F32 && a->dtype != LNX_BF16)) return -1;
+    GemmP p;
+    fill_gemm_p(a, p);
+    return nt_choose(p, a->dtype, a->out_f32 != 0).f;
 }
 
 extern "C" int lnx_gemm_nt(const lnx_gemm_args* a, void* stream) {
diff --git a/linnaeus_amd/csrc/plan.cpp b/linnaeus_amd/csrc/plan.cpp
--- a/linnaeus_amd/csrc/plan.cpp
+++ b/linnaeus_amd/csrc/plan.cpp
@@ -127,6 +127,9 @@
     int freq_pending = 0;
     bool freq_defer = true;
     bool ln_defer = true;
+    bool cm_ln_from_y = true;
+    bool dw_y16 = true;
+    int64_t o_g16 = 0;
     int64_t o_tnws = 0;
     int64_t o_lsws = 0, lsws_floats = 0;
     int64_t o_gcos , o_delta, o_dt1, o_tail[6], o_mtmp[4], o_dlT;
@@ -361,6 +364,8 @@
     p->esz = c.dtype == LNX_BF16 ? 2 : 4;
     p->meta_chain = !env_off("LNX_META_CHAIN");
     p->ln_defer = !env_off("LNX_LN_DEFER");
+    p->cm_ln_from_y = !env_off("LNX_CM_LN_FROM_Y");
+    p->dw_y16 = !env_off("LNX_DW_Y16");
     p->freq_defer = !env_off("LNX_FREQ_DEFER");
     for (int s = 0; s < 2; ++s) p->chain_ok[s] = p->meta_chain && lnx_meta_heads_supported(c.dims[2 + s]) != 0;
     p->E = 1 + c.n_meta;
@@ -604,6 +609,8 @@
         if (any_fused) p->o_sB = cv.take(maxM4C * esz);
         p->o_sC = cv.take(maxMC * esz);
         p->o_sD = cv.take(maxMC * esz);
+        const int64_t mc1 = (int64_t)B * p->HW[1] * D[1];
+        if (p->dw_y16 && esz == 2 && c.conv_depths[1] > 0 && maxMC >= 2 * mc1) p->o_g16 = p->o_sC + mc1 * esz;
     }
     if (!inf) {
         int64_t gmax = 0, dmax = 0;
@@ -1509,7 +1516,7 @@
     return 0;
 }
 
-int conv_block_bwd(const Ctx& c, int s, int i, float* g) {
+int conv_block_bwd(const Ctx& c, int s, int i, float* g, void* g16 = nullptr) {
     lnx_plan* p = c.p;
     ConvBlk& k = p->conv[s][i];
     const int B = p->c.batch, H = p->H[s], W = p->W[s], C = p->c.dims[s];
@@ -1524,14 +1531,14 @@
         lnx_convmlp_bwd_args f;
         memset(&f, 0, sizeof f);
         f.dtype = c.dt; f.M = M; f.C = C;
-        f.g = g; f.ln = c.at<void>(k.ln); f.w1 = c.wptr(k.w1); f.b1 = p->P[k.b1];
+        f.g = g; f.ln = k.fused_ln && p->cm_ln_from_y && C > 96 ? nullptr : c.at<void>(k.ln); f.w1 = c.wptr(k.w1); f.b1 = p->P[k.b1];
         f.w2t = c.wtptr(k.w2); f.w1t = c.wtptr(k.w1); f.gamma = p->P[k.gamma];
         f.rowscale = p->drop_ptr(p->drop_conv[s][i]); f.rows_per_sample = H * W;
         f.act = sB; f.dh = sA; f.dz = sC; f.dln = sD; f.dgamma = p->G[k.gamma];
         f.dz_plain = 1;
         if (k.fused_ln) {
             f.y = c.at<void>(k.y); f.ln_w = p->P[k.lnw]; f.mean = c.at<float>(k.mean); f.rstd = c.at<float>(k.rstd);
-            f.d_ln_w = p->G[k.lnw]; f.d_ln_b = p->G[k.lnb];
+            f.d_ln_w = p->G[k.lnw]; f.d_ln_b = p->G[k.lnb]; f.ln_b = p->P[k.lnb];
             f.ws = c.at<float>(p->o_lnws); f.ws_floats = p->lnws_floats;
             if (p->ln_defer && p->o_lnws_defer != 0 && lnx_convmlp_bwd_ws_floats(C, M) <= p->lnws_defer_floats) {
                 RUN(ln_defer_slot(c, f.ws, f.ws_floats));
@@ -1584,7 +1591,7 @@
     lnx_dwconv_args d;
     memset(&d, 0, sizeof d);
     d.B = B; d.H = H; d.W = W; d.C = C;
-    d.x = dy; d.x_dtype = c.dt; d.w49 = c.at<float>(k.w49); d.bias = nullptr; d.flip = 1; d.res = g; d.y = g; d.y_dtype = LNX_F32;
+    d.x = dy; d.x_dtype = c.dt; d.w49 = c.at<float>(k.w49); d.bias = nullptr; d.flip = 1; d.res = g; d.y = g; d.y_dtype = LNX_F32; d.y16 = g16;
     {
         Timed t(c, 4, (double)M * C * (8 + p->esz));
         RUN(lnx_dwconv7_fwd(&d, c.st));
@@ -1594,25 +1601,28 @@
 }
 
 int downsample_bwd(const Ctx& c, int i, const float* gout, int64_t ldg, lnx_rowmap gmap, const void* x, int xdt, int64_t ldx, lnx_rowmap xm, void* dx, int dxdt,
-                   int64_t lddx) {
+                   int64_t lddx, const void* dy16 = nullptr) {
     lnx_plan* p = c.p;
     Down& d = p->down[i];
     const int B = p->c.batch, Hin = p->H[i], Win = p->W[i], Cin = p->c.dims[i], Cout = p->c.dims[i + 1];
     const int Min = B * Hin * Win, Mout = Min / 4;
     void* sA = c.at<void>(p->o_sA);
-    void* sC = c.at<void>(p->o_sC);
-    RUN(lnx_scale_cast(gout, ldg, gmap, nullptr, 0, sC, c.dt, Cout, Mout, Cout, c.st));
+    const void* dY = dy16;
+    if (!dY) {
+        RUN(lnx_scale_cast(gout, ldg, gmap, nullptr, 0, c.at<void>(p->o_sC), c.dt, Cout, Mout, Cout, c.st));
+        dY = c.at<void>(p->o_sC);
+    }
     lnx_wgrad_args w;
     memset(&w, 0, sizeof w);
     w.dtype = c.dt; w.M = Mout; w.N = Cout; w.K = 4 * Cin;
-    w.dY = sC; w.lddy = Cout; w.A = c.at<void>(d.ln); w.a_mode = LNX_ADDR_PATCH2; w.Hin = Hin; w.Win = Win; w.Cin = Cin;
+    w.dY = dY; w.lddy = Cout; w.A = c.at<void>(d.ln); w.a_mode = LNX_ADDR_PATCH2; w.Hin = Hin; w.Win = Win; w.Cin = Cin;
     w.dW = p->G[d.w.param]; w.lddw = 4 * Cin; w.k_perm_c = Cin; w.db = p->G[d.cb];
     w.ws = c.at<float>(p->o_tnws); w.ws_floats = LNX_TN_WS_FLOATS;
     {
         Timed t(c, 1, 2.0 * Mout * Cout * 4 * Cin);
         RUN(lnx_gemm_tn(&w, c.st));
     }
-    lnx_gemm_args a = gemm_base(c, Mout, 4 * Cin, Cout, sC, Cout, c.wtptr(d.w), d.w.ld_t, sA, 0, false);
+    lnx_gemm_args a = gemm_base(c, Mout, 4 * Cin, Cout, dY, Cout, c.wtptr(d.w), d.w.ld_t, sA, 0, false);
     a.c_mode = LNX_ADDR_PATCH2; a.Hin = Hin; a.Win = Win; a.Cin = Cin;
     RUN(gemm_nt_t(c, &a));
     RUN(ln_bwd(c, Min, Cin, sA, c.dt, Cin, IDM, x, xdt, ldx, xm, d.lnw, d.lnb, c.at<float>(d.mean), c.at<float>(d.rstd), nullptr, dx, dxdt, lddx, false));
@@ -1824,11 +1834,12 @@
     }
     if (all || segment == 2) {
         float* g1 = c.at<float>(p->o_g[1]);
+        void* g16 = p->o_g16 != 0 && cf.conv_depths[1] > 0 ? c.at<void>(p->o_g16) : nullptr;
         for (int i = cf.conv_depths[1] - 1; i >= 0; --i) {
             RUN(conv_block_restore(c, 1, i));
-            RUN(conv_block_bwd(c, 1, i, g1));
-        }
-        RUN(downsample_bwd(c, 0, g1, D[1], IDM, c.at<float>(p->o_stage_out[0]), LNX_F32, D[0], IDM, c.at<float>(p->o_g[0]), LNX_F32, D[0]));
+            RUN(conv_block_bwd(c, 1, i, g1, i == 0 ? g16 : nullptr));
+        }
+        RUN(downsample_bwd(c, 0, g1, D[1], IDM, c.at<float>(p->o_stage_out[0]), LNX_F32, D[0], IDM, c.at<float>(p->o_g[0]), LNX_F32, D[0], g16));
         RUN(ln_flush(c));
         RUN(join_side(c, 0));
     }
diff --git a/linnaeus_amd/ops.py b/linnaeus_amd/ops.py
--- a/linnaeus_amd/ops.py
+++ b/linnaeus_amd/ops.py
@@ -228,12 +228,12 @@
     L.check(L.lib().lnx_layernorm_bwd_flush(_stream()), "lnx_layernorm_bwd_flush")
 
 
-def dwconv7(x, w49, bias, y, *, flip=False, res=None):
+def dwconv7(x, w49, bias, y, *, flip=False, res=None, y16=None):
     B, H, W, Cc = x.shape
     a = L.DwconvArgs()
     a.B, a.H, a.W, a.C = B, H, W, Cc
     a.x, a.x_dtype, a.w49, a.bias = _p(x), code_of(x), _p(w49), _p(bias)
-    a.flip, a.res, a.y, a.y_dtype = int(flip), _p(res), _p(y), code_of(y)
+    a.flip, a.res, a.y, a.y_dtype, a.y16 = int(flip), _p(res), _p(y), code_of(y), _p(y16)
     L.check(L.lib().lnx_dwconv7_fwd(C.byref(a), _stream()), "lnx_dwconv7_fwd")
     return y
 
@@ -382,15 +382,16 @@
 
 
 def convmlp_bwd(g, ln, z, w1, b1, w2t, w1t, gamma, act, dh, dz, dln, dgamma, *, rowscale=None, rows_per_sample=0, y=None, ln_w=None, mean=None,
-                rstd=None, d_ln_w=None, d_ln_b=None, ws=None, dz_plain=False):
+                rstd=None, d_ln_w=None, d_ln_b=None, ws=None, dz_plain=False, ln_b=None, ln_defer=False):
     a = L.ConvMlpBwdArgs()
-    a.dtype, a.M, a.C = code_of(ln), ln.shape[0], ln.shape[1]
+    src = ln if ln is not None else y
+    a.dtype, a.M, a.C = code_of(src), src.shape[0], src.shape[1]
     a.g, a.ln, a.z, a.w1, a.b1, a.w2t, a.w1t, a.gamma = _p(g), _p(ln), _p(z), _p(w1), _p(b1), _p(w2t), _p(w1t), _p(gamma)
     a.rowscale, a.rows_per_sample = _p(rowscale), rows_per_sample
     a.act, a.dh, a.dz, a.dln, a.dgamma = _p(act), _p(dh), _p(dz), _p(dln), _p(dgamma)
     a.y, a.ln_w, a.mean, a.rstd, a.d_ln_w, a.d_ln_b = _p(y), _p(ln_w), _p(mean), _p(rstd), _p(d_ln_w), _p(d_ln_b)
     a.ws, a.ws_floats = _p(ws), (ws.numel() if ws is not None else 0)
-    a.dz_plain = int(dz_plain)
+    a.dz_plain, a.ln_defer, a.ln_b = int(dz_plain), int(ln_defer), _p(ln_b)
     L.check(L.lib().lnx_convmlp_bwd(C.byref(a), _stream()), "lnx_convmlp_bwd")
 
 
```
